# darskkaa/NTIRE-2026-Light-Field-Image-Super-Resolution-Challenge---Track-2-Efficiency

Measured on AMD Instinct MI355X. Metric: 5x5 x4-SR LF patches/sec (32^2->128^2), DistgSSR inference, higher is better.
Workload: dtype f32 (EPI branch stage 1 / 2 and fuse.0: fp32 operands as three exact bf16 terms on the bf16 MFMA pipe, six products, fp32 accumulation -- error against fp64 not above the fp32-MFMA kernels', tests/test_gpu_b3_accuracy.py; 3x3 convs, angular branch, init, head: fp32 MFMA)

## Files before the change

### include/lfsr_hip.h

```cpp
#ifndef LFSR_HIP_H
#define LFSR_HIP_H

#include <stddef.h>
#include <stdint.h>

#ifdef __cplusplus
extern "C" {
#endif

#define LFSR_OK 0
#define LFSR_E_ARG (-1)
#define LFSR_E_WS (-2)

const char* lfsr_version(void);


int lfsr_sai2macpi(const void* in, void* out, int B, int C, int A, int h, int w, int elem_bytes, void* stream);
int lfsr_macpi2sai(const void* in, void* out, int B, int C, int A, int h, int w, int elem_bytes, void* stream);
int lfsr_pixel_shuffle2d(const void* in, void* out, int B, int C, int r, int H, int W, int elem_bytes, void* stream);
int lfsr_pixel_shuffle1d(const void* in, void* out, int B, int C, int f, int H, int W, int elem_bytes, void* stream);
int lfsr_image_extend(const void* in, void* out, int N, int h, int w, int top, int bottom, int left, int right,
                      int elem_bytes, void* stream);
int lfsr_lf_divide(const void* in, void* out, int A, int h0, int w0, int P, int S, int elem_bytes,
                   int* num_u, int* num_v, void* stream);
int lfsr_lf_integrate(const void* in, void* out, int A, int numU, int numV, int pz, int stride, int h, int w,
                      int elem_bytes, void* stream);

int lfsr_lf_crop_tiles(const void* in, void* tiles, int A, int count, int pz, int stride, int elem_bytes, void* stream);
int lfsr_lf_place_tiles(const void* tiles, void* out, int A, int numU, int numV, int first, int count, int stride, int h, int w,
                        int elem_bytes, void* stream);

int lfsr_nchw_to_vcl(const float* in, float* out, int out_stride, int out_choff, int B, int C, int A, int h, int w,
                     int layout, void* stream);
int lfsr_vcl_to_nchw(const float* in, int in_stride, int in_choff, float* out, int B, int C, int A, int h, int w,
                     int layout, void* stream);


int lfsr_pack_conv_weight(const float* w, float* packed, int O, int C, int taps, int perm, int ch, void* stream);
size_t lfsr_packed_weight_floats(int O, int C, int taps);

int lfsr_conv3x3_fwd(const float* x, int x_stride, int x_choff, const float* w_packed,
                     float* y, int y_stride, int y_choff,
                     const float* r1, int r1_stride, int r1_choff, const float* r2, int r2_stride, int r2_choff,
                     int n_img, int h, int w, float slope, void* stream);

int lfsr_pointwise_fwd(const float* x, int x_stride, int x_choff, int cin, const float* w_packed, const float* bias,
                       float* y, int y_stride, int y_choff, int M, int N, float slope, void* stream);

int lfsr_angconv_fwd(const float* x, int x_stride, int x_choff, const float* w1_packed, const float* w2_packed,
                     float* tmp, float* y, int y_stride, int y_choff, int B, int A, int h, int w, float slope, void* stream);

int lfsr_epiconv_fwd(const float* x, int x_stride, int x_choff, const float* w1_packed, const float* w2_packed,
                     float* tmp, float* y, int y_stride, int y_choff, int B, int A, int h, int w, int vertical,
                     float slope, void* stream);

int lfsr_epiconv_hv_fwd(const float* x, int x_stride, int x_choff, const float* w1_packed, const float* w2_packed,
                        float* tmp, float* y, int y_stride, int choff_h, int choff_v, int B, int A, int h, int w,
                        float slope, void* stream);

int lfsr_initconv_fwd(const float* x, const float* w, float* y, int y_stride, int y_choff, int B, int A, int h, int wd,
                      void* stream);

int lfsr_fold_head(const float* w0, const float* b0, const float* w2, float* wf, float* bf, int C, int s, void* stream);
int lfsr_upsample_head_fwd(const float* f, int f_stride, int f_choff, const float* wf, const float* bf,
                           const float* x_lr, float* out, int B, int A, int h, int w, int s, void* stream);

typedef struct lfsr_distgssr lfsr_distgssr;

int lfsr_distgssr_create(lfsr_distgssr** ctx, int A, int scale, int n_group, int n_block, int channels);
void lfsr_distgssr_destroy(lfsr_distgssr* ctx);
size_t lfsr_distgssr_packed_bytes(const lfsr_distgssr* ctx);
int lfsr_distgssr_set_packed(lfsr_distgssr* ctx, void* packed, size_t bytes);
int lfsr_distgssr_load_param(lfsr_distgssr* ctx, const char* key, const float* data, size_t numel, void* stream);
int lfsr_distgssr_finalize(lfsr_distgssr* ctx, void* stream);
int lfsr_distgssr_begin_batched_load(lfsr_distgssr* ctx);
size_t lfsr_distgssr_workspace_bytes(const lfsr_distgssr* ctx, int B, int h, int w);
int lfsr_distgssr_forward(lfsr_distgssr* ctx, const float* x, float* out, int B, int h, int w,
                          void* workspace, size_t workspace_bytes, void* stream);
int lfsr_distgssr_forward_taps(lfsr_distgssr* ctx, const float* x, float* out, int B, int h, int w,
                               void* workspace, size_t workspace_bytes, float* const* taps, void* stream);

size_t lfsr_distgssr_num_params(const lfsr_distgssr* ctx);
int lfsr_distgssr_param_offset(const lfsr_distgssr* ctx, const char* key, size_t* offset, size_t* numel);
size_t lfsr_distgssr_train_workspace_bytes(const lfsr_distgssr* ctx, int B, int h, int w);
int lfsr_distgssr_forward_train(lfsr_distgssr* ctx, const float* x, float* out, int B, int h, int w,
                                void* workspace, size_t workspace_bytes, void* stream);
int lfsr_distgssr_train_saved(const lfsr_distgssr* ctx, int B, int h, int w, int which, int index, size_t* offset_floats, size_t* numel);
int lfsr_distgssr_backward(lfsr_distgssr* ctx, const float* x, const float* dout, int B, int h, int w,
                           void* workspace, size_t workspace_bytes, float* grads, size_t n_grads, void* stream);

size_t lfsr_packed_weight_tr_floats(int O, int C, int taps);
int lfsr_pack_conv_weight_tr(const float* w, float* packed_T, int O, int C, int taps, void* stream);
int lfsr_conv3x3_dgrad(const float* dy, int dy_stride, int dy_choff, const float* wT_packed, float* dx, int dx_stride, int dx_choff,
                       const float* r1, int r1_stride, int r1_choff, const float* act, int act_stride, int act_choff, float act_slope,
                       int n_img, int h, int w, void* stream);
size_t lfsr_conv3x3_wgrad_workspace_floats(int n_img, int h, int w);
int lfsr_conv3x3_wgrad(const float* dy, int dy_stride, int dy_choff, const float* x, int x_stride, int x_choff, float* dw,
                       float* workspace, size_t workspace_floats, int n_img, int h, int w, int accumulate, void* stream);
int lfsr_pointwise_dgrad(const float* dy, int dy_stride, int dy_choff, int cout, const float* wT_packed, float* dx, int dx_stride, int dx_choff, int cin,
                         const float* act, int act_stride, int act_choff, float act_slope, long long M, void* stream);
size_t lfsr_pointwise_wgrad_workspace_floats(long long M, int cout, int cin);
int lfsr_pointwise_wgrad(const float* dy, int dy_stride, int dy_choff, int cout, const float* x, int x_stride, int x_choff, int cin, float* dw,
                         float* workspace, size_t workspace_floats, long long M, int accumulate, void* stream);
int lfsr_upsample_head_dgrad(const float* dout, const float* wf, float* df, float* g16, int B, int A, int h, int w, int s, void* stream);

int lfsr_comm_available(void);
int lfsr_comm_unique_id(void* id128);
int lfsr_comm_init(void** comm, int world, int rank, const void* id128);
int lfsr_comm_destroy(void* comm);
int lfsr_allreduce(void* grads, size_t n, void* comm, void* stream);

#define LFSR_DISTG_NCLASS 6
int lfsr_distgssr_profile(lfsr_distgssr* ctx, int enable);
int lfsr_distgssr_profile_read(lfsr_distgssr* ctx, double* ms, long long* launches);

int lfsr_layernorm_fwd(const float* x, int x_stride, int x_choff, const float* pe, int pe_stride, long long pe_rows, long long pe_div,
                       const float* gamma, const float* beta, float* y, int y_stride, int y_choff, long long M, int C,
                       float eps, void* stream);
int lfsr_linear_fwd(const float* x, int x_stride, int x_choff, int cin, const float* w_packed, const float* bias,
                    const float* res, int res_stride, int res_choff, float* y, int y_stride, int y_choff,
                    long long M, int N, float slope, void* stream);
int lfsr_ffn_fwd(const float* x, int x_stride, int x_choff, const float* w1_packed, const float* w2_packed,
                 const float* res, int res_stride, int res_choff, float* y, int y_stride, int y_choff,
                 long long M, int K1, int H, int N2, float slope, void* stream);
int lfsr_ffn_ln_fwd(const float* x, int x_stride, int x_choff, const float* gamma, const float* beta, float eps,
                    const float* w1_packed, const float* w2_packed, const float* res, int res_stride, int res_choff,
                    float* y, int y_stride, int y_choff, long long M, int K1, int H, int N2, float slope, void* stream);
int lfsr_linear_ln_fwd(const float* x, int x_stride, int x_choff, int K, const float* w_packed, const float* gamma, const float* beta,
                       float eps, int ln_cols, const float* pe, int pe_stride, int pe_rows, int pe_div,
                       float* y, int y_stride, int y_choff, float* y2, int y2_stride, int y2_choff, int split_n,
                       long long M, int N, void* stream);
int lfsr_window_attn_fwd(const float* q, int q_stride, int q_choff, const float* k, int k_stride, int k_choff,
                         const float* v, int v_stride, int v_choff, float* o, int o_stride, int o_choff, int nheads, int hd,
                         int ns0, int ns1, int ns2, long long bs0, long long bs1, long long bs2,
                         int n1, int n2, long long st1, long long st2, int l1, int r1, int l2, int r2, int clip2, void* stream);
int lfsr_conv3x3_n_fwd(const float* x, int x_stride, int x_choff, const float* w_packed, float* y, int y_stride, int y_choff,
                       int n_img, int h, int w, int N, float slope, void* stream);
int lfsr_lft_position_fwd(float* spa_pe, float* ang_pe, int A, int h, int w, int C, void* stream);
int lfsr_upsample_ps_fwd(const float* f, int f_stride, int f_choff, const float* w_packed, float* hr, int B, int A, int h, int w,
                         int s, void* stream);
int lfsr_up_tail_fwd(const float* f, int f_stride, int f_choff, const float* w0_packed, const float* w3, const float* x_lr, float* out,
                     int B, int A, int h, int w, int s, float slope, void* stream);
int lfsr_hr_tail_fwd(const float* hr, const float* w3, const float* x_lr, float* out, int B, int A, int h, int w, int s,
                     float slope, void* stream);

typedef struct lfsr_epit lfsr_epit;
int lfsr_epit_create(lfsr_epit** ctx, int A, int scale, int n_block, int channels);
void lfsr_epit_destroy(lfsr_epit* ctx);
size_t lfsr_epit_packed_bytes(const lfsr_epit* ctx);
int lfsr_epit_set_packed(lfsr_epit* ctx, void* packed, size_t bytes);
int lfsr_epit_load_param(lfsr_epit* ctx, const char* key, const float* data, size_t numel, void* stream);
int lfsr_epit_finalize(lfsr_epit* ctx, void* stream);
size_t lfsr_epit_workspace_bytes(const lfsr_epit* ctx, int B, int h, int w);
int lfsr_epit_forward(lfsr_epit* ctx, const float* x, float* out, int B, int h, int w, void* workspace, size_t workspace_bytes,
                      void* stream);

typedef struct lfsr_lft lfsr_lft;
int lfsr_lft_create(lfsr_lft** ctx, int A, int scale, int n_layer, int channels);
void lfsr_lft_destroy(lfsr_lft* ctx);
size_t lfsr_lft_packed_bytes(const lfsr_lft* ctx);
int lfsr_lft_set_packed(lfsr_lft* ctx, void* packed, size_t bytes);
int lfsr_lft_load_param(lfsr_lft* ctx, const char* key, const float* data, size_t numel, void* stream);
int lfsr_lft_finalize(lfsr_lft* ctx, void* stream);
size_t lfsr_lft_workspace_bytes(const lfsr_lft* ctx, int B, int h, int w);
int lfsr_lft_forward(lfsr_lft* ctx, const float* x, float* out, int B, int h, int w, void* workspace, size_t workspace_bytes,
                     void* stream);

int lfsr_view_metrics(const float* label, const float* out, double* psnr, double* ssim, int B, int A, int H, int W, void* stream);
int lfsr_mask_views(const float* x, float* y, const unsigned char* mask, float fill, int B, int C, int A, int h, int w, void* stream);
int lfsr_mask_views_fill(const float* x, float* y, const unsigned char* mask, const float* fill, int B, int C, int A, int h, int w, void* stream);

int lfsr_ycbcr2rgb_views(const float* y, const float* cbcr, unsigned char* out, int A, int h, int w, const double* minv255,
                         const double* offset, void* stream);

typedef struct lfsr_internet lfsr_internet;
int lfsr_internet_create(lfsr_internet** ctx, int A, int scale, int n_groups, int n_layers);
void lfsr_internet_destroy(lfsr_internet* ctx);
size_t lfsr_internet_packed_bytes(const lfsr_internet* ctx);
int lfsr_internet_set_packed(lfsr_internet* ctx, void* packed, size_t bytes);
int lfsr_internet_load_param(lfsr_internet* ctx, const char* key, const float* data, size_t numel, void* stream);
int lfsr_internet_finalize(lfsr_internet* ctx, void* stream);
size_t lfsr_internet_workspace_bytes(const lfsr_internet* ctx, int B, int h, int w);
int lfsr_internet_forward(lfsr_internet* ctx, const float* x, float* out, int B, int h, int w, void* workspace,
                          size_t workspace_bytes, void* stream);

size_t lfsr_angconv_bwd_workspace_floats(int B, int A, int h, int w);
int lfsr_angconv_bwd(const float* dy, int dy_stride, int dy_choff, const float* y, int y_stride, int y_choff, const float* x, const float* a16,
                     const float* w0, const float* w2, float* dx, float* dw0, float* dw2, float* workspace, size_t workspace_floats,
                     int B, int A, int h, int w, float slope, void* stream);
size_t lfsr_epiconv_hv_bwd_workspace_floats(int B, int A, int h, int w);
int lfsr_epiconv_hv_bwd(const float* dy, int dy_stride, int choff_h, int choff_v, const float* y, int y_stride, int y_choff_h, int y_choff_v,
                        const float* x, const float* e_h, const float* e_v, const float* w0, const float* w2,
                        float* dx, float* dw0, float* dw2, float* workspace, size_t workspace_floats, int B, int A, int h, int w, float slope, void* stream);

#define LFSR_ARITH_DEFAULT 0
#define LFSR_ARITH_F32 1
int lfsr_set_arithmetic(int mode);
int lfsr_get_arithmetic(void);

int lfsr_op_profile(int enable);
long long lfsr_op_profile_read(char* buf, size_t cap);

#ifdef __cplusplus
}
#endif
#endif
```

### ntire-2026-light-field-image-super-resolution-challenge---track-2-efficiency_amd/capi.py

```python
import ctypes as C
import os

import torch

_HERE = os.path.dirname(os.path.abspath(__file__))
LIB_PATH = os.environ.get("LFSR_HIP_LIB") or os.path.join(_HERE, "liblfsr_hip.so")

c_p = C.c_void_p
c_i = C.c_int
c_f = C.c_float
c_sz = C.c_size_t

SIGNATURES = {
    "lfsr_version": (C.c_char_p, []),
    "lfsr_sai2macpi": (c_i, [c_p, c_p, c_i, c_i, c_i, c_i, c_i, c_i, c_p]),
    "lfsr_macpi2sai": (c_i, [c_p, c_p, c_i, c_i, c_i, c_i, c_i, c_i, c_p]),
    "lfsr_pixel_shuffle2d": (c_i, [c_p, c_p, c_i, c_i, c_i, c_i, c_i, c_i, c_p]),
    "lfsr_pixel_shuffle1d": (c_i, [c_p, c_p, c_i, c_i, c_i, c_i, c_i, c_i, c_p]),
    "lfsr_image_extend": (c_i, [c_p, c_p, c_i, c_i, c_i, c_i, c_i, c_i, c_i, c_i, c_p]),
    "lfsr_lf_divide": (c_i, [c_p, c_p, c_i, c_i, c_i, c_i, c_i, c_i, C.POINTER(c_i), C.POINTER(c_i), c_p]),
    "lfsr_lf_integrate": (c_i, [c_p, c_p, c_i, c_i, c_i, c_i, c_i, c_i, c_i, c_i, c_p]),
    "lfsr_lf_crop_tiles": (c_i, [c_p, c_p, c_i, c_i, c_i, c_i, c_i, c_p]),
    "lfsr_lf_place_tiles": (c_i, [c_p, c_p, c_i, c_i, c_i, c_i, c_i, c_i, c_i, c_i, c_i, c_p]),
    "lfsr_nchw_to_vcl": (c_i, [c_p, c_p, c_i, c_i, c_i, c_i, c_i, c_i, c_i, c_i, c_p]),
    "lfsr_vcl_to_nchw": (c_i, [c_p, c_i, c_i, c_p, c_i, c_i, c_i, c_i, c_i, c_i, c_p]),
    "lfsr_pack_conv_weight": (c_i, [c_p, c_p, c_i, c_i, c_i, c_i, c_i, c_p]),
    "lfsr_packed_weight_floats": (c_sz, [c_i, c_i, c_i]),
    "lfsr_conv3x3_fwd": (c_i, [c_p, c_i, c_i, c_p, c_p, c_i, c_i, c_p, c_i, c_i, c_p, c_i, c_i, c_i, c_i, c_i, c_f, c_p]),
    "lfsr_pointwise_fwd": (c_i, [c_p, c_i, c_i, c_i, c_p, c_p, c_p, c_i, c_i, c_i, c_i, c_f, c_p]),
    "lfsr_angconv_fwd": (c_i, [c_p, c_i, c_i, c_p, c_p, c_p, c_p, c_i, c_i, c_i, c_i, c_i, c_i, c_f, c_p]),
    "lfsr_epiconv_fwd": (c_i, [c_p, c_i, c_i, c_p, c_p, c_p, c_p, c_i, c_i, c_i, c_i, c_i, c_i, c_i, c_f, c_p]),
    "lfsr_epiconv_hv_fwd": (c_i, [c_p, c_i, c_i, c_p, c_p, c_p, c_p, c_i, c_i, c_i, c_i, c_i, c_i, c_i, c_f, c_p]),
    "lfsr_initconv_fwd": (c_i, [c_p, c_p, c_p, c_i, c_i, c_i, c_i, c_i, c_i, c_p]),
    "lfsr_fold_head": (c_i, [c_p, c_p, c_p, c_p, c_p, c_i, c_i, c_p]),
    "lfsr_upsample_head_fwd": (c_i, [c_p, c_i, c_i, c_p, c_p, c_p, c_p, c_i, c_i, c_i, c_i, c_i, c_p]),
    "lfsr_distgssr_create": (c_i, [C.POINTER(c_p), c_i, c_i, c_i, c_i, c_i]),
    "lfsr_distgssr_destroy": (None, [c_p]),
    "lfsr_distgssr_packed_bytes": (c_sz, [c_p]),
    "lfsr_distgssr_set_packed": (c_i, [c_p, c_p, c_sz]),
    "lfsr_distgssr_load_param": (c_i, [c_p, C.c_char_p, c_p, c_sz, c_p]),
    "lfsr_distgssr_finalize": (c_i, [c_p, c_p]),
    "lfsr_distgssr_begin_batched_load": (c_i, [c_p]),
    "lfsr_distgssr_workspace_bytes": (c_sz, [c_p, c_i, c_i, c_i]),
    "lfsr_distgssr_forward": (c_i, [c_p, c_p, c_p, c_i, c_i, c_i, c_p, c_sz, c_p]),
    "lfsr_distgssr_forward_taps": (c_i, [c_p, c_p, c_p, c_i, c_i, c_i, c_p, c_sz, C.POINTER(c_p), c_p]),
    "lfsr_distgssr_num_params": (c_sz, [c_p]),
    "lfsr_distgssr_param_offset": (c_i, [c_p, C.c_char_p, C.POINTER(c_sz), C.POINTER(c_sz)]),
    "lfsr_distgssr_train_workspace_bytes": (c_sz, [c_p, c_i, c_i, c_i]),
    "lfsr_distgssr_forward_train": (c_i, [c_p, c_p, c_p, c_i, c_i, c_i, c_p, c_sz, c_p]),
    "lfsr_distgssr_train_saved": (c_i, [c_p, c_i, c_i, c_i, c_i, c_i, C.POINTER(c_sz), C.POINTER(c_sz)]),
    "lfsr_distgssr_backward": (c_i, [c_p, c_p, c_p, c_i, c_i, c_i, c_p, c_sz, c_p, c_sz, c_p]),
    "lfsr_layernorm_fwd": (c_i, [c_p, c_i, c_i, c_p, c_i, C.c_longlong, C.c_longlong, c_p, c_p, c_p, c_i, c_i, C.c_longlong, c_i, c_f, c_p]),
    "lfsr_conv3x3_n_fwd": (c_i, [c_p, c_i, c_i, c_p, c_p, c_i, c_i, c_i, c_i, c_i, c_i, c_f, c_p]),
    "lfsr_lft_position_fwd": (c_i, [c_p, c_p, c_i, c_i, c_i, c_i, c_p]),
    "lfsr_view_metrics": (c_i, [c_p, c_p, c_p, c_p, c_i, c_i, c_i, c_i, c_p]),
    "lfsr_mask_views": (c_i, [c_p, c_p, c_p, c_f, c_i, c_i, c_i, c_i, c_i, c_p]),
    "lfsr_mask_views_fill": (c_i, [c_p, c_p, c_p, c_p, c_i, c_i, c_i, c_i, c_i, c_p]),
    "lfsr_internet_create": (c_i, [C.POINTER(c_p), c_i, c_i, c_i, c_i]),
    "lfsr_internet_destroy": (None, [c_p]),
    "lfsr_internet_packed_bytes": (c_sz, [c_p]),
    "lfsr_internet_set_packed": (c_i, [c_p, c_p, c_sz]),
    "lfsr_internet_load_param": (c_i, [c_p, C.c_char_p, c_p, c_sz, c_p]),
    "lfsr_internet_finalize": (c_i, [c_p, c_p]),
    "lfsr_internet_workspace_bytes": (c_sz, [c_p, c_i, c_i, c_i]),
    "lfsr_internet_forward": (c_i, [c_p, c_p, c_p, c_i, c_i, c_i, c_p, c_sz, c_p]),
    "lfsr_lft_create": (c_i, [C.POINTER(c_p), c_i, c_i, c_i, c_i]),
    "lfsr_lft_destroy": (None, [c_p]),
    "lfsr_lft_packed_bytes": (c_sz, [c_p]),
    "lfsr_lft_set_packed": (c_i, [c_p, c_p, c_sz]),
    "lfsr_lft_load_param": (c_i, [c_p, C.c_char_p, c_p, c_sz, c_p]),
    "lfsr_lft_finalize": (c_i, [c_p, c_p]),
    "lfsr_lft_workspace_bytes": (c_sz, [c_p, c_i, c_i, c_i]),
    "lfsr_lft_forward": (c_i, [c_p, c_p, c_p, c_i, c_i, c_i, c_p, c_sz, c_p]),
    "lfsr_linear_fwd": (c_i, [c_p, c_i, c_i, c_i, c_p, c_p, c_p, c_i, c_i, c_p, c_i, c_i, C.c_longlong, c_i, c_f, c_p]),
    "lfsr_ycbcr2rgb_views": (c_i, [c_p, c_p, c_p, c_i, c_i, c_i, C.POINTER(C.c_double), C.POINTER(C.c_double), c_p]),
    "lfsr_ffn_fwd": (c_i, [c_p, c_i, c_i, c_p, c_p, c_p, c_i, c_i, c_p, c_i, c_i, C.c_longlong, c_i, c_i, c_i, c_f, c_p]),
    "lfsr_ffn_ln_fwd": (c_i, [c_p, c_i, c_i, c_p, c_p, c_f, c_p, c_p, c_p, c_i, c_i, c_p, c_i, c_i, C.c_longlong, c_i, c_i, c_i, c_f, c_p]),
    "lfsr_linear_ln_fwd": (c_i, [c_p, c_i, c_i, c_i, c_p, c_p, c_p, c_f, c_i, c_p, c_i, c_i, c_i, c_p, c_i, c_i, c_p, c_i, c_i, c_i, C.c_longlong, c_i, c_p]),
    "lfsr_window_attn_fwd": (c_i, [c_p, c_i, c_i, c_p, c_i, c_i, c_p, c_i, c_i, c_p, c_i, c_i, c_i, c_i, c_i, c_i, c_i,
                                   C.c_longlong, C.c_longlong, C.c_longlong, c_i, c_i, C.c_longlong, C.c_longlong, c_i, c_i, c_i, c_i, c_i, c_p]),
    "lfsr_upsample_ps_fwd": (c_i, [c_p, c_i, c_i, c_p, c_p, c_i, c_i, c_i, c_i, c_i, c_p]),
    "lfsr_up_tail_fwd": (c_i, [c_p, c_i, c_i, c_p, c_p, c_p, c_p, c_i, c_i, c_i, c_i, c_i, c_f, c_p]),
    "lfsr_hr_tail_fwd": (c_i, [c_p, c_p, c_p, c_p, c_i, c_i, c_i, c_i, c_i, c_f, c_p]),
    "lfsr_epit_create": (c_i, [C.POINTER(c_p), c_i, c_i, c_i, c_i]),
    "lfsr_epit_destroy": (None, [c_p]),
    "lfsr_epit_packed_bytes": (c_sz, [c_p]),
    "lfsr_epit_set_packed": (c_i, [c_p, c_p, c_sz]),
    "lfsr_epit_load_param": (c_i, [c_p, C.c_char_p, c_p, c_sz, c_p]),
    "lfsr_epit_finalize": (c_i, [c_p, c_p]),
    "lfsr_epit_workspace_bytes": (c_sz, [c_p, c_i, c_i, c_i]),
    "lfsr_epit_forward": (c_i, [c_p, c_p, c_p, c_i, c_i, c_i, c_p, c_sz, c_p]),
    "lfsr_packed_weight_tr_floats": (c_sz, [c_i, c_i, c_i]),
    "lfsr_pack_conv_weight_tr": (c_i, [c_p, c_p, c_i, c_i, c_i, c_p]),
    "lfsr_conv3x3_dgrad": (c_i, [c_p, c_i, c_i, c_p, c_p, c_i, c_i, c_p, c_i, c_i, c_p, c_i, c_i, c_f, c_i, c_i, c_i, c_p]),
    "lfsr_conv3x3_wgrad_workspace_floats": (c_sz, [c_i, c_i, c_i]),
    "lfsr_conv3x3_wgrad": (c_i, [c_p, c_i, c_i, c_p, c_i, c_i, c_p, c_p, c_sz, c_i, c_i, c_i, c_i, c_p]),
    "lfsr_pointwise_dgrad": (c_i, [c_p, c_i, c_i, c_i, c_p, c_p, c_i, c_i, c_i, c_p, c_i, c_i, c_f, C.c_longlong, c_p]),
    "lfsr_pointwise_wgrad_workspace_floats": (c_sz, [C.c_longlong, c_i, c_i]),
    "lfsr_pointwise_wgrad": (c_i, [c_p, c_i, c_i, c_i, c_p, c_i, c_i, c_i, c_p, c_p, c_sz, C.c_longlong, c_i, c_p]),
    "lfsr_upsample_head_dgrad": (c_i, [c_p, c_p, c_p, c_p, c_i, c_i, c_i, c_i, c_i, c_p]),
    "lfsr_comm_available": (c_i, []),
    "lfsr_comm_unique_id": (c_i, [c_p]),
    "lfsr_comm_init": (c_i, [C.POINTER(c_p), c_i, c_i, c_p]),
    "lfsr_comm_destroy": (c_i, [c_p]),
    "lfsr_allreduce": (c_i, [c_p, c_sz, c_p, c_p]),
    "lfsr_angconv_bwd_workspace_floats": (c_sz, [c_i, c_i, c_i, c_i]),
    "lfsr_angconv_bwd": (c_i, [c_p, c_i, c_i, c_p, c_i, c_i, c_p, c_p, c_p, c_p, c_p, c_p, c_p, c_p, c_sz, c_i, c_i, c_i, c_i, c_f, c_p]),
    "lfsr_epiconv_hv_bwd_workspace_floats": (c_sz, [c_i, c_i, c_i, c_i]),
    "lfsr_epiconv_hv_bwd": (c_i, [c_p, c_i, c_i, c_i, c_p, c_i, c_i, c_i, c_p, c_p, c_p, c_p, c_p, c_p, c_p, c_p, c_p, c_sz, c_i, c_i, c_i, c_i, c_f, c_p]),
    "lfsr_set_arithmetic": (c_i, [c_i]),
    "lfsr_get_arithmetic": (c_i, []),
    "lfsr_op_profile": (c_i, [c_i]),
    "lfsr_op_profile_read": (C.c_longlong, [C.c_char_p, c_sz]),
    "lfsr_distgssr_profile": (c_i, [c_p, c_i]),
    "lfsr_distgssr_profile_read": (c_i, [c_p, C.POINTER(C.c_double), C.POINTER(C.c_longlong)]),
}

_lib = None


class LfsrError(RuntimeError):
    pass


def load():
    global _lib
    if _lib is None:
        if not os.path.exists(LIB_PATH):
            raise LfsrError(f"{LIB_PATH} not built: run `python -c 'import __graft_entry__ as g; g.build()'` "
                            "(there is no CPU fallback for the HIP path)")
        lib = C.CDLL(LIB_PATH)
        for name, (res, args) in SIGNATURES.items():
            fn = getattr(lib, name)
            fn.restype = res
            fn.argtypes = args
        _lib = lib
    return _lib


def check(rc, what):
    if rc != 0:
        if rc == -1:
            msg = "bad argument"
        elif rc == -2:
            msg = "workspace too small"
        else:
            msg = f"HIP error {-rc - 1000}"
        raise LfsrError(f"{what}: {msg} (rc={rc})")


def stream_ptr():
    return C.c_void_p(torch.cuda.current_stream().cuda_stream)


def dev_ptr(t, what="tensor"):
    if not isinstance(t, torch.Tensor) or not t.is_cuda:
        raise LfsrError(f"{what} must be a CUDA/ROCm tensor: the HIP path has no CPU fallback")
    if not t.is_contiguous():
        raise LfsrError(f"{what} must be contiguous")
    return C.c_void_p(t.data_ptr())


def _elem(t):
    eb = t.element_size()
    if eb not in (2, 4):
        raise LfsrError(f"unsupported element size {eb}")
    return eb


ARITH_DEFAULT, ARITH_F32 = 0, 1


def set_arithmetic(mode):
    check(load().lfsr_set_arithmetic(int(mode)), "set_arithmetic")


def op_profile(enable):
    check(load().lfsr_op_profile(int(bool(enable))), "op_profile")


def op_profile_read():
    lib = load()
    cap = 1 << 18
    buf = C.create_string_buffer(cap)
    need = lib.lfsr_op_profile_read(buf, cap)
    if need < 0:
        check(int(need), "op_profile_read")
    if need > cap:
        raise LfsrError(f"op_profile_read: table of {need} bytes truncated")
    out = {}
    for line in buf.value.decode().splitlines():
        op, a, b, ms, n = line.split()
        out[(op, int(a), int(b))] = (float(ms), int(n))
    return out



def sai2macpi(x, A):
    lib = load()
    B, Cc, Hh, Ww = x.shape
    out = torch.empty_like(x)
    check(lib.lfsr_sai2macpi(dev_ptr(x), dev_ptr(out), B, Cc, A, Hh // A, Ww // A, _elem(x), stream_ptr()), "sai2macpi")
    return out


def macpi2sai(x, A):
    lib = load()
    B, Cc, Hh, Ww = x.shape
    out = torch.empty_like(x)
    check(lib.lfsr_macpi2sai(dev_ptr(x), dev_ptr(out), B, Cc, A, Hh // A, Ww // A, _elem(x), stream_ptr()), "macpi2sai")
    return out


def pixel_shuffle2d(x, r):
    lib = load()
    B, Crr, H, W = x.shape
    Cc = Crr // (r * r)
    out = torch.empty((B, Cc, H * r, W * r), dtype=x.dtype, device=x.device)
    check(lib.lfsr_pixel_shuffle2d(dev_ptr(x), dev_ptr(out), B, Cc, r, H, W, _elem(x), stream_ptr()), "pixel_shuffle2d")
    return out


def pixel_shuffle1d(x, f):
    lib = load()
    B, fC, H, W = x.shape
    Cc = fC // f
    out = torch.empty((B, Cc, H, W * f), dtype=x.dtype, device=x.device)
    check(lib.lfsr_pixel_shuffle1d(dev_ptr(x), dev_ptr(out), B, Cc, f, H, W, _elem(x), stream_ptr()), "pixel_shuffle1d")
    return out


def image_extend(im, bdr):
    lib = load()
    h, w = im.shape[-2:]
    N = im.numel() // (h * w) if h * w else 0
    out = torch.empty(tuple(im.shape[:-2]) + (h + bdr[0] + bdr[1], w + bdr[2] + bdr[3]), dtype=im.dtype, device=im.device)
    check(lib.lfsr_image_extend(dev_ptr(im), dev_ptr(out), N, h, w, bdr[0], bdr[1], bdr[2], bdr[3], _elem(im), stream_ptr()), "image_extend")
    return out


def lf_divide(data, A, P, S):
    lib = load()
    if data.dim() != 2:
        raise LfsrError("LFdivide expects a 2-D (A*h0, A*w0) mosaic")
    h0, w0 = data.shape[0] // A, data.shape[1] // A
    nu, nv = c_i(0), c_i(0)
    check(lib.lfsr_lf_divide(None, None, A, h0, w0, P, S, _elem(data), C.byref(nu), C.byref(nv), None), "lf_divide(count)")
    out = torch.empty((nu.value, nv.value, A * P, A * P), dtype=data.dtype, device=data.device)
    check(lib.lfsr_lf_divide(dev_ptr(data), dev_ptr(out), A, h0, w0, P, S, _elem(data), None, None, stream_ptr()), "lf_divide")
    return out


def lf_integrate(sub, A, pz, stride, h, w):
    lib = load()
    if sub.dim() == 6:
        n1, n2 = sub.shape[:2]
        sub = sub.permute(0, 1, 2, 4, 3, 5).reshape(n1, n2, A * pz, A * pz).contiguous()
    n1, n2 = sub.shape[:2]
    out = torch.empty((A, A, h, w), dtype=sub.dtype, device=sub.device)
    check(lib.lfsr_lf_integrate(dev_ptr(sub), dev_ptr(out), A, n1, n2, pz, stride, h, w, _elem(sub), stream_ptr()), "lf_integrate")
    return out


def lf_crop_tiles(sub, A, pz, stride):
    lib = load()
    n = sub.shape[0]
    if sub.shape[-1] != A * pz or sub.shape[-2] != A * pz or sub.numel() != n * A * pz * A * pz:
        raise LfsrError(f"lf_crop_tiles: bad patch tensor {tuple(sub.shape)} for A={A} pz={pz}")
    sub = sub.contiguous()
    out = torch.empty((n, A, A, stride, stride), dtype=sub.dtype, device=sub.device)
    check(lib.lfsr_lf_crop_tiles(dev_ptr(sub), dev_ptr(out), A, n, pz, stride, _elem(sub), stream_ptr()), "lf_crop_tiles")
    return out


def lf_place_tiles(tiles, out, A, numU, numV, first, stride):
    lib = load()
    tiles = tiles.contiguous()
    if not out.is_contiguous() or out.dtype != tiles.dtype or out.shape[0] != A or out.shape[1] != A:
        raise LfsrError("lf_place_tiles: bad output tensor")
    check(lib.lfsr_lf_place_tiles(dev_ptr(tiles), dev_ptr(out), A, numU, numV, first, tiles.shape[0], stride, out.shape[2], out.shape[3], _elem(tiles), stream_ptr()),
          "lf_place_tiles")
    return out


def nchw_to_vcl(x, A, layout, out=None, choff=0):
    lib = load()
    B, Cc, Hh, Ww = x.shape
    h, w = Hh // A, Ww // A
    if out is None:
        out = torch.empty((B * A * A * h * w, Cc), dtype=torch.float32, device=x.device)
    check(lib.lfsr_nchw_to_vcl(dev_ptr(x), dev_ptr(out), out.shape[1], choff, B, Cc, A, h, w, layout, stream_ptr()), "nchw_to_vcl")
    return out


def vcl_to_nchw(v, B, Cc, A, h, w, layout, choff=0):
    lib = load()
    out = torch.empty((B, Cc, A * h, A * w), dtype=torch.float32, device=v.device)
    check(lib.lfsr_vcl_to_nchw(dev_ptr(v), v.shape[1], choff, dev_ptr(out), B, Cc, A, h, w, layout, stream_ptr()), "vcl_to_nchw")
    return out


def pack_conv_weight(w, perm=0, ch=0):
    lib = load()
    O, Cc = w.shape[:2]
    taps = w.numel() // (O * Cc)
    n = lib.lfsr_packed_weight_floats(O, Cc, taps)
    out = torch.empty(n, dtype=torch.float32, device=w.device)
    check(lib.lfsr_pack_conv_weight(dev_ptr(w), dev_ptr(out), O, Cc, taps, perm, ch, stream_ptr()), "pack_conv_weight")
    return out



def max_patches_per_launch(A, h, w, widest_row_floats, limit=1 << 31):
    per_patch = A * A * h * w * widest_row_floats * 4
    return max(1, (limit - 1) // per_patch)


def _forward_in_chunks(fwd, x, nmax):
    return torch.cat([fwd(x[i:i + nmax]) for i in range(0, x.shape[0], nmax)], 0)


class GraphedForward:

    def __init__(self, rt):
        self.rt = rt
        self.graphs = {}

    def __call__(self, x):
        key = (tuple(x.shape), x.device, x.dtype)
        g = self.graphs.get(key)
        if g is None:
            static_x = x.clone()
            side = torch.cuda.Stream(device=x.device)
            side.wait_stream(torch.cuda.current_stream())
            with torch.cuda.stream(side):
                for _ in range(2):
                    self.rt.forward(static_x)
            torch.cuda.current_stream().wait_stream(side)
            graph = torch.cuda.CUDAGraph()
            with torch.cuda.graph(graph):
                static_y = self.rt.forward(static_x)
            g = self.graphs[key] = (graph, static_x, static_y)
        graph, static_x, static_y = g
        static_x.copy_(x)
        graph.replay()
        return static_y



class DistgSSRRuntime:

    def __init__(self, A, scale, n_group=4, n_block=4, channels=64):
        self.lib = load()
        self.A, self.scale = A, scale
        ctx = c_p()
        check(self.lib.lfsr_distgssr_create(C.byref(ctx), A, scale, n_group, n_block, channels), "distgssr_create")
        self.ctx = ctx
        self.packed = None
        self.ws = {}
        self.loaded_version = None
        self.train_generation = 0

    def __del__(self):
        try:
            if getattr(self, "ctx", None):
                self.lib.lfsr_distgssr_destroy(self.ctx)
                self.ctx = None
        except Exception:
            pass

    def load_state(self, named_tensors, device, fanout=None, batched=False):
        nbytes = self.lib.lfsr_distgssr_packed_bytes(self.ctx)
        if self.packed is None or self.packed.device != device:
            self.packed = torch.empty(nbytes, dtype=torch.uint8, device=device)
        check(self.lib.lfsr_distgssr_set_packed(self.ctx, dev_ptr(self.packed), nbytes), "distgssr_set_packed")
        cur = torch.cuda.current_stream(device)
        st = stream_ptr()
        keep = []
        if batched:
            check(self.lib.lfsr_distgssr_begin_batched_load(self.ctx), "distgssr_begin_batched_load")
        if fanout:
            fork = torch.cuda.Event()
            fork.record(cur)
            for s in fanout:
                s.wait_event(fork)
        for i, (k, t) in enumerate(named_tensors):
            t = t.detach()
            if t.dtype != torch.float32:
                t = t.float()
            t = t.contiguous()
            sp = C.c_void_p(fanout[i % len(fanout)].cuda_stream) if fanout else st
            keep.append(t)
            check(self.lib.lfsr_distgssr_load_param(self.ctx, k.encode(), dev_ptr(t, k), t.numel(), sp), f"distgssr_load_param({k})")
        if fanout:
            for s in fanout:
                e = torch.cuda.Event()
                e.record(s)
                cur.wait_event(e)
        check(self.lib.lfsr_distgssr_finalize(self.ctx, st), "distgssr_finalize")

    def _workspace(self, B, h, w, device):
        key = (B, h, w, device)
        if key not in self.ws:
            self.ws.clear()
            n = self.lib.lfsr_distgssr_workspace_bytes(self.ctx, B, h, w)
            self.ws[key] = torch.empty(n, dtype=torch.uint8, device=device)
        return self.ws[key]

    def num_params(self):
        return self.lib.lfsr_distgssr_num_params(self.ctx)

    def param_span(self, key):
        off, n = c_sz(0), c_sz(0)
        check(self.lib.lfsr_distgssr_param_offset(self.ctx, key.encode(), C.byref(off), C.byref(n)), f"param_offset({key})")
        return off.value, n.value

    def _train_workspace(self, B, h, w, device):
        key = ("train", B, h, w, device)
        if key not in self.ws:
            self.ws.clear()
            n = self.lib.lfsr_distgssr_train_workspace_bytes(self.ctx, B, h, w)
            self.ws[key] = torch.empty(n, dtype=torch.uint8, device=device)
        return self.ws[key]

    def forward_train(self, x):
        B, c1, Hh, Ww = x.shape
        if c1 != 1 or Hh % self.A or Ww % self.A or x.dtype != torch.float32:
            raise LfsrError(f"bad training input {tuple(x.shape)} {x.dtype}")
        h, w = Hh // self.A, Ww // self.A
        x = x.contiguous()
        out = torch.empty((B, 1, Hh * self.scale, Ww * self.scale), dtype=torch.float32, device=x.device)
        ws = self._train_workspace(B, h, w, x.device)
        check(self.lib.lfsr_distgssr_forward_train(self.ctx, dev_ptr(x), dev_ptr(out), B, h, w, dev_ptr(ws), ws.numel(), stream_ptr()),
              "distgssr_forward_train")
        self.train_generation += 1
        return out

    def backward(self, x, dout, grads=None):
        B, _, Hh, Ww = x.shape
        h, w = Hh // self.A, Ww // self.A
        n = self.num_params()
        if grads is None:
            grads = torch.empty(n, dtype=torch.float32, device=x.device)
        ws = self._train_workspace(B, h, w, x.device)
        dout = dout.contiguous()
        if dout.dtype != torch.float32:
            dout = dout.float()
        check(self.lib.lfsr_distgssr_backward(self.ctx, dev_ptr(x.contiguous()), dev_ptr(dout), B, h, w, dev_ptr(ws), ws.numel(),
                                              dev_ptr(grads), n, stream_ptr()), "distgssr_backward")
        return grads

    def train_saved(self, x, which, index):
        B, _, Hh, Ww = x.shape
        h, w = Hh // self.A, Ww // self.A
        off, n = c_sz(0), c_sz(0)
        check(self.lib.lfsr_distgssr_train_saved(self.ctx, B, h, w, which, index, C.byref(off), C.byref(n)), "train_saved")
        ws = self._train_workspace(B, h, w, x.device).view(torch.float32)
        return ws[off.value:off.value + n.value]

    PROFILE_CLASSES = ("conv3x3", "angconv", "epiconv", "pointwise", "init_conv", "upsample_head")

    def profile(self, enable):
        check(self.lib.lfsr_distgssr_profile(self.ctx, int(enable)), "distgssr_profile")

    def profile_read(self):
        ms = (C.c_double * 6)()
        n = (C.c_longlong * 6)()
        check(self.lib.lfsr_distgssr_profile_read(self.ctx, ms, n), "distgssr_profile_read")
        return {k: (ms[i], n[i]) for i, k in enumerate(self.PROFILE_CLASSES)}

    def forward(self, x, taps=None):
        B, c1, Hh, Ww = x.shape
        if c1 != 1 or Hh % self.A or Ww % self.A:
            raise LfsrError(f"bad input shape {tuple(x.shape)} for angRes {self.A}")
        if x.dtype != torch.float32:
            raise LfsrError("DistgSSR HIP path computes in fp32; got " + str(x.dtype))
        h, w = Hh // self.A, Ww // self.A
        x = x.contiguous()
        if taps is None and B > max_patches_per_launch(self.A, h, w, 160, 1 << 30):
            return _forward_in_chunks(self.forward, x, max_patches_per_launch(self.A, h, w, 160, 1 << 30))
        out = torch.empty((B, 1, Hh * self.scale, Ww * self.scale), dtype=torch.float32, device=x.device)
        ws = self._workspace(B, h, w, x.device)
        if taps is None:
            check(self.lib.lfsr_distgssr_forward(self.ctx, dev_ptr(x), dev_ptr(out), B, h, w, dev_ptr(ws), ws.numel(), stream_ptr()),
                  "distgssr_forward")
            return out
        bufs = []
        arr = (c_p * 5)()
        for i in range(5):
            if taps[i]:
                t = torch.empty((B, 144 if i == 4 else 64, Hh, Ww), dtype=torch.float32, device=x.device)
                arr[i] = t.data_ptr()
            else:
                t = None
                arr[i] = None
            bufs.append(t)
        check(self.lib.lfsr_distgssr_forward_taps(self.ctx, dev_ptr(x), dev_ptr(out), B, h, w, dev_ptr(ws), ws.numel(), arr, stream_ptr()),
              "distgssr_forward_taps")
        return out, bufs



def _opt(t):
    return dev_ptr(t) if t is not None else None


def conv3x3(x, w_packed, n_img, h, w, slope=1.0, res1=None, res2=None, out=None, out_choff=0, x_choff=0):
    lib = load()
    if out is None:
        out = torch.empty((n_img * h * w, 64), dtype=torch.float32, device=x.device)
    check(lib.lfsr_conv3x3_fwd(dev_ptr(x), x.shape[1], x_choff, dev_ptr(w_packed), dev_ptr(out), out.shape[1], out_choff,
                               _opt(res1), res1.shape[1] if res1 is not None else 0, 0,
                               _opt(res2), res2.shape[1] if res2 is not None else 0, 0,
                               n_img, h, w, slope, stream_ptr()), "conv3x3_fwd")
    return out


def pointwise(x, cin, w_packed, N, slope=1.0, bias=None, out=None, out_choff=0, x_choff=0):
    lib = load()
    M = x.shape[0]
    if out is None:
        out = torch.empty((M, N), dtype=torch.float32, device=x.device)
    check(lib.lfsr_pointwise_fwd(dev_ptr(x), x.shape[1], x_choff, cin, dev_ptr(w_packed), _opt(bias), dev_ptr(out), out.shape[1], out_choff,
                                 M, N, slope, stream_ptr()), "pointwise_fwd")
    return out


def angconv(x, w1p, w2p, B, A, h, w, slope, out, out_choff, tmp=None):
    lib = load()
    if tmp is None:
        tmp = torch.empty((B * h * w, 16), dtype=torch.float32, device=x.device)
    check(lib.lfsr_angconv_fwd(dev_ptr(x), x.shape[1], 0, dev_ptr(w1p), dev_ptr(w2p), dev_ptr(tmp), dev_ptr(out), out.shape[1], out_choff,
                               B, A, h, w, slope, stream_ptr()), "angconv_fwd")
    return out


def epiconv(x, w1p, w2p, B, A, h, w, vertical, slope, out, out_choff, tmp=None):
    lib = load()
    if tmp is None:
        tmp = torch.empty((B * A * h * w, 32), dtype=torch.float32, device=x.device)
    check(lib.lfsr_epiconv_fwd(dev_ptr(x), x.shape[1], 0, dev_ptr(w1p), dev_ptr(w2p), dev_ptr(tmp), dev_ptr(out), out.shape[1], out_choff,
                               B, A, h, w, int(vertical), slope, stream_ptr()), "epiconv_fwd")
    return out


def epiconv_hv(x, w1p, w2p, B, A, h, w, slope, out, choff_h, choff_v):
    lib = load()
    tmp = torch.empty((B * A * h * w, 32), dtype=torch.float32, device=x.device)
    check(lib.lfsr_epiconv_hv_fwd(dev_ptr(x), x.shape[1], 0, dev_ptr(w1p), dev_ptr(w2p), dev_ptr(tmp), dev_ptr(out), out.shape[1], choff_h, choff_v,
                                  B, A, h, w, slope, stream_ptr()), "epiconv_hv_fwd")
    return out


def initconv(x, w, A):
    lib = load()
    B, _, Hh, Ww = x.shape
    h, wd = Hh // A, Ww // A
    out = torch.empty((B * A * A * h * wd, 64), dtype=torch.float32, device=x.device)
    check(lib.lfsr_initconv_fwd(dev_ptr(x), dev_ptr(w), dev_ptr(out), 64, 0, B, A, h, wd, stream_ptr()), "initconv_fwd")
    return out


def upsample_head(f, w0, b0, w2, x_lr, A, s):
    lib = load()
    B, _, Hh, Ww = x_lr.shape
    h, w = Hh // A, Ww // A
    wf = torch.empty(s * s * 64, dtype=torch.float32, device=f.device)
    bf = torch.empty(s * s, dtype=torch.float32, device=f.device)
    check(lib.lfsr_fold_head(dev_ptr(w0), _opt(b0), dev_ptr(w2), dev_ptr(wf), dev_ptr(bf), 64, s, stream_ptr()), "fold_head")
    out = torch.empty((B, 1, Hh * s, Ww * s), dtype=torch.float32, device=f.device)
    check(lib.lfsr_upsample_head_fwd(dev_ptr(f), f.shape[1], 0, dev_ptr(wf), dev_ptr(bf), dev_ptr(x_lr), dev_ptr(out), B, A, h, w, s, stream_ptr()),
          "upsample_head_fwd")
    return out



class ModelRuntime:

    def __init__(self, name, A, scale, *create_args):
        self.lib = load()
        self.name, self.A, self.scale = name, A, scale
        self._f = lambda fn: getattr(self.lib, f"lfsr_{name}_{fn}")
        ctx = c_p()
        check(self._f("create")(C.byref(ctx), A, scale, *create_args), f"{name}_create")
        self.ctx = ctx
        self.packed = None
        self.ws = {}

    def __del__(self):
        try:
            if getattr(self, "ctx", None):
                self._f("destroy")(self.ctx)
                self.ctx = None
        except Exception:
            pass

    def load_state(self, named_tensors, device):
        nbytes = self._f("packed_bytes")(self.ctx)
        if self.packed is None or self.packed.device != device:
            self.packed = torch.empty(nbytes, dtype=torch.uint8, device=device)
        check(self._f("set_packed")(self.ctx, dev_ptr(self.packed), nbytes), f"{self.name}_set_packed")
        st = stream_ptr()
        for k, t in named_tensors:
            t = t.detach().float().contiguous()
            check(self._f("load_param")(self.ctx, k.encode(), dev_ptr(t, k), t.numel(), st), f"{self.name}_load_param({k})")
        check(self._f("finalize")(self.ctx, st), f"{self.name}_finalize")

    def forward(self, x):
        B, c1, Hh, Ww = x.shape
        if c1 != 1 or Hh % self.A or Ww % self.A:
            raise LfsrError(f"bad input shape {tuple(x.shape)} for angRes {self.A}")
        if x.dtype != torch.float32:
            raise LfsrError(f"{self.name} HIP path computes in fp32; got {x.dtype}")
        h, w = Hh // self.A, Ww // self.A
        x = x.contiguous()
        if B > max_patches_per_launch(self.A, h, w, 256):
            return _forward_in_chunks(self.forward, x, max_patches_per_launch(self.A, h, w, 256))
        out = torch.empty((B, 1, Hh * self.scale, Ww * self.scale), dtype=torch.float32, device=x.device)
        key = (B, h, w, x.device)
        if key not in self.ws:
            self.ws.clear()
            self.ws[key] = torch.empty(self._f("workspace_bytes")(self.ctx, B, h, w), dtype=torch.uint8, device=x.device)
        ws = self.ws[key]
        check(self._f("forward")(self.ctx, dev_ptr(x), dev_ptr(out), B, h, w, dev_ptr(ws), ws.numel(), stream_ptr()), f"{self.name}_forward")
        return out



def pack_conv_weight_T(w):
    lib = load()
    O, Cc = w.shape[:2]
    taps = w.numel() // (O * Cc)
    out = torch.empty(lib.lfsr_packed_weight_tr_floats(O, Cc, taps), dtype=torch.float32, device=w.device)
    check(lib.lfsr_pack_conv_weight_tr(dev_ptr(w), dev_ptr(out), O, Cc, taps, stream_ptr()), "pack_conv_weight_T")
    return out


def conv3x3_dgrad(dy, wT_packed, n_img, h, w, res1=None, act=None, act_slope=1.0):
    lib = load()
    dx = torch.empty((n_img * h * w, 64), dtype=torch.float32, device=dy.device)
    check(lib.lfsr_conv3x3_dgrad(dev_ptr(dy), dy.shape[1], 0, dev_ptr(wT_packed), dev_ptr(dx), 64, 0,
                                 _opt(res1), res1.shape[1] if res1 is not None else 0, 0,
                                 _opt(act), act.shape[1] if act is not None else 0, 0, act_slope, n_img, h, w, stream_ptr()), "conv3x3_dgrad")
    return dx


def conv3x3_wgrad(dy, x, n_img, h, w, dw=None):
    lib = load()
    acc = dw is not None
    if dw is None:
        dw = torch.empty((64, 64, 3, 3), dtype=torch.float32, device=dy.device)
    ws = torch.empty(lib.lfsr_conv3x3_wgrad_workspace_floats(n_img, h, w), dtype=torch.float32, device=dy.device)
    check(lib.lfsr_conv3x3_wgrad(dev_ptr(dy), dy.shape[1], 0, dev_ptr(x), x.shape[1], 0, dev_ptr(dw), dev_ptr(ws), ws.numel(), n_img, h, w, int(acc),
                                 stream_ptr()), "conv3x3_wgrad")
    return dw


def pointwise_dgrad(dy, wT_packed, cin, act=None, act_slope=1.0):
    lib = load()
    M = dy.shape[0]
    dx = torch.empty((M, cin), dtype=torch.float32, device=dy.device)
    check(lib.lfsr_pointwise_dgrad(dev_ptr(dy), dy.shape[1], 0, 64, dev_ptr(wT_packed), dev_ptr(dx), cin, 0, cin,
                                   _opt(act), act.shape[1] if act is not None else 0, 0, act_slope, M, stream_ptr()), "pointwise_dgrad")
    return dx


def pointwise_wgrad(dy, x, cout, cin):
    lib = load()
    M = dy.shape[0]
    dw = torch.empty((cout, cin), dtype=torch.float32, device=dy.device)
    ws = torch.empty(lib.lfsr_pointwise_wgrad_workspace_floats(M, cout, cin), dtype=torch.float32, device=dy.device)
    check(lib.lfsr_pointwise_wgrad(dev_ptr(dy), dy.shape[1], 0, cout, dev_ptr(x), x.shape[1], 0, cin, dev_ptr(dw), dev_ptr(ws), ws.numel(), M, 0,
                                   stream_ptr()), "pointwise_wgrad")
    return dw


class RcclComm:

    def __init__(self, world, rank, exchange=None):
        self.lib = load()
        if not self.lib.lfsr_comm_available():
            raise LfsrError("RCCL not found (librccl.so): lfsr_allreduce is unavailable on this host")
        buf = C.create_string_buffer(128)
        if rank == 0:
            check(self.lib.lfsr_comm_unique_id(buf), "comm_unique_id")
        raw = bytes(buf.raw)
        if world > 1:
            if exchange is None:
                raise LfsrError("world > 1 needs an `exchange` callable to ship rank 0's unique id")
            raw = exchange(raw)
        comm = c_p()
        check(self.lib.lfsr_comm_init(C.byref(comm), world, rank, C.create_string_buffer(raw, 128)), "comm_init")
        self.comm, self.world = comm, world

    def allreduce_(self, t):
        if t.dtype != torch.float32:
            raise LfsrError("lfsr_allreduce carries fp32 buckets")
        check(self.lib.lfsr_allreduce(dev_ptr(t), t.numel(), self.comm, stream_ptr()), "allreduce")
        return t

    def close(self):
        if getattr(self, "comm", None):
            self.lib.lfsr_comm_destroy(self.comm)
            self.comm = None


def angconv_bwd(dy, dy_choff, y, y_choff, x, a16, w0, w2, dx, B, A, h, w, slope=0.1):
    lib = load()
    ws = torch.empty(lib.lfsr_angconv_bwd_workspace_floats(B, A, h, w), dtype=torch.float32, device=x.device)
    dw0, dw2 = torch.empty_like(w0), torch.empty_like(w2)
    check(lib.lfsr_angconv_bwd(dev_ptr(dy), dy.shape[1], dy_choff, _opt(y), y.shape[1] if y is not None else 0, y_choff, dev_ptr(x), dev_ptr(a16),
                               dev_ptr(w0.contiguous()), dev_ptr(w2.contiguous()), dev_ptr(dx), dev_ptr(dw0), dev_ptr(dw2), dev_ptr(ws), ws.numel(), B, A, h, w, slope,
                               stream_ptr()), "angconv_bwd")
    return dw0, dw2


def epiconv_hv_bwd(dy, choff_h, choff_v, y, y_choff_h, y_choff_v, x, e_h, e_v, w0, w2, dx, B, A, h, w, slope=0.1):
    lib = load()
    ws = torch.empty(lib.lfsr_epiconv_hv_bwd_workspace_floats(B, A, h, w), dtype=torch.float32, device=x.device)
    dw0, dw2 = torch.empty_like(w0), torch.empty_like(w2)
    check(lib.lfsr_epiconv_hv_bwd(dev_ptr(dy), dy.shape[1], choff_h, choff_v, _opt(y), y.shape[1] if y is not None else 0, y_choff_h, y_choff_v, dev_ptr(x),
                                  dev_ptr(e_h), dev_ptr(e_v), dev_ptr(w0.contiguous()), dev_ptr(w2.contiguous()), dev_ptr(dx), dev_ptr(dw0), dev_ptr(dw2),
                                  dev_ptr(ws), ws.numel(), B, A, h, w, slope, stream_ptr()), "epiconv_hv_bwd")
    return dw0, dw2
```

### ntire-2026-light-field-image-super-resolution-challenge---track-2-efficiency_amd/csrc/ang_fused.hip

```cpp
#include "lfsr_internal.h"

typedef float f32x4a __attribute__((ext_vector_type(4)));

namespace {

constexpr int W1ROW = 68;
constexpr int TROW = 20;

struct AngArgs {
  const float* X; int x_stride; int x_choff;
  const float* W1;
  const float* W2;
  float* T;
  float* Y; int y_stride; int y_choff;
  int B, A, H, W;
  float slope;
};

__global__ __launch_bounds__(512) void k_ang_fused(AngArgs p) {
  extern __shared__ __attribute__((aligned(16))) float sm[];
  const int AA = p.A * p.A, HW = p.H * p.W, M = p.B * HW;
  float* sW1 = sm;
  float* sW2 = sm + AA * 16 * W1ROW;
  float* sT = sW2 + 16 * AA * 16;
  const int tid = threadIdx.x, lane = tid & 63, wave = tid >> 6, nwave = blockDim.x >> 6;
  const int i = lane & 15, kq = lane >> 4;

  const int ngroups = (M + 15) / 16, gstride = (int)gridDim.x * nwave;
  const int g0 = (int)blockIdx.x * nwave + wave;
  const long long tstep = (long long)HW * p.x_stride;
  float4 fb[2][5][4];
  auto load_row = [&](int g, int u, float4 (*f)[4]) {
    const int m = g * 16 + i;
    const bool ok = m < M;
    const int mb = ok ? m / HW : 0, myx = ok ? m - mb * HW : 0;
    const float* src = p.X + ((long long)mb * AA * HW + myx) * p.x_stride + p.x_choff + 4 * kq;
#pragma unroll
    for (int v = 0; v < 5; ++v)
#pragma unroll
      for (int j = 0; j < 4; ++j)
        f[v][j] = (ok && v < p.A) ? *reinterpret_cast<const float4*>(src + (u * p.A + v) * tstep + 16 * j) : make_float4(0.f, 0.f, 0.f, 0.f);
  };
  {
    float4 wv[13];
#pragma unroll
    for (int q = 0; q < 13; ++q) {
      const int idx = tid + q * 512, row = idx >> 4, c = idx & 15, tap = row >> 4, n = row & 15;
      wv[q] = idx < AA * 256 ? *reinterpret_cast<const float4*>(p.W1 + ((long long)tap * 32 + n) * 64 + c * 4) : make_float4(0.f, 0.f, 0.f, 0.f);
    }
    float4 w2v[4];
#pragma unroll
    for (int q = 0; q < 4; ++q) {
      const int idx = tid + q * 512;
      w2v[q] = idx < AA * 64 ? reinterpret_cast<const float4*>(p.W2)[idx] : make_float4(0.f, 0.f, 0.f, 0.f);
    }
    if (g0 < ngroups) load_row(g0, 0, fb[0]);
#pragma unroll
    for (int q = 0; q < 13; ++q) {
      const int idx = tid + q * 512;
      if (idx < AA * 256) *reinterpret_cast<float4*>(sW1 + (idx >> 4) * W1ROW + (idx & 15) * 4) = wv[q];
    }
#pragma unroll
    for (int q = 0; q < 4; ++q) {
      const int idx = tid + q * 512;
      if (idx < AA * 64) reinterpret_cast<float4*>(sW2)[idx] = w2v[q];
    }
  }
  __syncthreads();

  float* st = sT + wave * 16 * TROW;
  const float* b1 = sW1 + i * W1ROW + 4 * kq;
  const float* b2 = sW2 + i * 16 + 4 * kq;

  for (int g = g0; g < ngroups; g += gstride) {
    const int m = g * 16 + i;
    const bool ok = m < M;
    const int mb = ok ? m / HW : 0, myx = ok ? m - mb * HW : 0;
    if (g != g0) load_row(g, 0, fb[0]);
    f32x4a acc = {0.f, 0.f, 0.f, 0.f};
#pragma unroll
    for (int u = 0; u < 5; ++u) {
      if (u >= p.A) break;
      if (u + 1 < p.A) load_row(g, u + 1, fb[(u + 1) & 1]);
#pragma unroll
      for (int v = 0; v < 5; ++v) {
        if (v >= p.A) break;
        const float* bt = b1 + (u * p.A + v) * 16 * W1ROW;
#pragma unroll
        for (int j = 0; j < 4; ++j) {
          const float4 b = *reinterpret_cast<const float4*>(bt + 16 * j);
          const float4 a = fb[u & 1][v][j];
          acc = __builtin_amdgcn_mfma_f32_16x16x4f32(a.x, b.x, acc, 0, 0, 0);
          acc = __builtin_amdgcn_mfma_f32_16x16x4f32(a.y, b.y, acc, 0, 0, 0);
          acc = __builtin_amdgcn_mfma_f32_16x16x4f32(a.z, b.z, acc, 0, 0, 0);
          acc = __builtin_amdgcn_mfma_f32_16x16x4f32(a.w, b.w, acc, 0, 0, 0);
        }
      }
    }
#pragma unroll
    for (int r = 0; r < 4; ++r) {
      float v = acc[r];
      v = v >= 0.f ? v : v * p.slope;
      st[(4 * kq + r) * TROW + i] = v;
    }
    const int b_i = ok ? mb : 0;
    const long long dbase = ok ? (long long)b_i * AA * HW + myx : -1;
    __builtin_amdgcn_wave_barrier();
    const float4 a2 = *reinterpret_cast<const float4*>(st + i * TROW + 4 * kq);
    if (ok) *reinterpret_cast<float4*>(p.T + (long long)m * 16 + 4 * kq) = a2;
    __builtin_amdgcn_wave_barrier();
    for (int view = 0; view < AA; ++view) {
      const float4 b = *reinterpret_cast<const float4*>(b2 + view * 256);
      f32x4a o = {0.f, 0.f, 0.f, 0.f};
      o = __builtin_amdgcn_mfma_f32_16x16x4f32(a2.x, b.x, o, 0, 0, 0);
      o = __builtin_amdgcn_mfma_f32_16x16x4f32(a2.y, b.y, o, 0, 0, 0);
      o = __builtin_amdgcn_mfma_f32_16x16x4f32(a2.z, b.z, o, 0, 0, 0);
      o = __builtin_amdgcn_mfma_f32_16x16x4f32(a2.w, b.w, o, 0, 0, 0);
#pragma unroll
      for (int r = 0; r < 4; ++r) {
        float v = o[r];
        v = v >= 0.f ? v : v * p.slope;
        st[(4 * kq + r) * TROW + i] = v;
      }
      __builtin_amdgcn_wave_barrier();
      const float4 z = *reinterpret_cast<const float4*>(st + i * TROW + 4 * kq);
      __builtin_amdgcn_wave_barrier();
      if (ok) *reinterpret_cast<float4*>(p.Y + (dbase + (long long)view * HW) * p.y_stride + p.y_choff + 4 * kq) = z;
    }
  }
}

}

size_t lfsr_ang_fused_smem(int A, int waves) {
  const int AA = A * A;
  return (size_t)(AA * 16 * W1ROW + 16 * AA * 16 + waves * 16 * TROW) * 4;
}

bool lfsr_ang_fused_ok(int A) { return A >= 1 && A <= 5 && lfsr_ang_fused_smem(A, 8) <= 160 * 1024; }

int lfsr_ang_fused_launch(const float* x, int x_stride, int x_choff, const float* w1_packed, const float* w2_packed, float* t, float* y,
                          int y_stride, int y_choff, int B, int A, int h, int w, float slope, hipStream_t st) {
  if (!lfsr_ang_fused_ok(A)) return LFSR_E_ARG;
  static std::atomic<bool> attr_set[64];
  int dev = 0;
  if (hipGetDevice(&dev) != hipSuccess || dev < 0 || dev >= 64) return LFSR_E_ARG;
  if (!attr_set[dev]) {
    hipError_t e = hipFuncSetAttribute(reinterpret_cast<const void*>(k_ang_fused), hipFuncAttributeMaxDynamicSharedMemorySize, 160 * 1024);
    if (e != hipSuccess) return LFSR_HIP_ERR(e);
    attr_set[dev] = true;
  }
  AngArgs p{};
  p.X = x; p.x_stride = x_stride; p.x_choff = x_choff; p.W1 = w1_packed; p.W2 = w2_packed; p.T = t;
  p.Y = y; p.y_stride = y_stride; p.y_choff = y_choff; p.B = B; p.A = A; p.H = h; p.W = w; p.slope = slope;
  const long long ngroups = ((long long)B * h * w + 15) / 16;
  const int waves = 8;
  long long grid = (ngroups + waves - 1) / waves;
  if (grid > 256) grid = 256;
  hipLaunchKernelGGL(k_ang_fused, dim3((unsigned)grid), dim3(waves * 64), lfsr_ang_fused_smem(A, waves), st, p);
  LFSR_CHECK_LAUNCH();
  return LFSR_OK;
}
```

### ntire-2026-light-field-image-super-resolution-challenge---track-2-efficiency_amd/csrc/distgssr.cpp

```cpp
#include <cstring>
#include <map>
#include <string>
#include <vector>

#include "lfsr_internal.h"

namespace {
struct Slot {
  size_t off = 0;
  size_t floats = 0;
  size_t numel = 0;
  int O = 0, C = 0, T = 0, perm = 0, ch = 0;
  bool raw = false, loaded = false;
  int kindT = 0;
  size_t offT = 0, floatsT = 0;
  size_t grad_off = 0;
};
inline size_t align64(size_t f) { return (f + 63) / 64 * 64; }
}

struct lfsr_distgssr {
  int A, s, G, NB, C;
  std::map<std::string, Slot> slots;
  std::vector<std::string> order;
  size_t n_params = 0;
  size_t packed_floats = 0, off_wf = 0, off_bf = 0;
  float* packed = nullptr;
  bool finalized = false;
  bool batch_mode = false;
  std::vector<LfsrPackDesc> d_gen, d_c3, d_epi, d_epib, uploaded;
  LfsrPackDesc* table_dev = nullptr;
  size_t table_cap = 0;
  hipStream_t side = nullptr;
  hipEvent_t ev_fork = nullptr, ev_join = nullptr, ev_a = nullptr, ev_b = nullptr;
  bool profiling = false;
  struct Ev { int cls; hipEvent_t a, b; };
  bool profile_all = true;
  int sample_stride = 1;
  long long sample_ctr = 0;
  std::vector<Ev> evs;
  std::vector<hipEvent_t> free_evs;
  hipEvent_t get_ev() {
    if (!free_evs.empty()) { hipEvent_t e = free_evs.back(); free_evs.pop_back(); return e; }
    hipEvent_t e = nullptr;
    (void)hipEventCreate(&e);
    return e;
  }

  void add(const std::string& k, int O, int Cc, int T, int perm, int ch, bool raw, int kindT = 0) {
    Slot sl;
    sl.O = O; sl.C = Cc; sl.T = T; sl.perm = perm; sl.ch = ch; sl.raw = raw; sl.kindT = kindT;
    sl.numel = (size_t)O * Cc * T;
    sl.floats = raw ? sl.numel : lfsr_packed_weight_floats(O, Cc, T);
    sl.off = packed_floats;
    packed_floats += align64(sl.floats);
    if (kindT == 1 || kindT == 2) sl.floatsT = (size_t)T * ((Cc + 31) / 32 * 32) * O;
    if (kindT == 1 && O == 64 && Cc == 64 && T == 9) sl.floatsT += LFSR_CONV3_WINO_FLOATS;
    if (kindT == 3 || kindT == 4) sl.floatsT = (size_t)(O / (kindT == 3 ? 16 : 32)) * ((Cc + 31) / 32 * 32) * (kindT == 3 ? 16 : 32);
    if (kindT) { sl.offT = packed_floats; packed_floats += align64(sl.floatsT); }
    sl.grad_off = n_params;
    n_params += sl.numel;
    slots[k] = sl;
    order.push_back(k);
  }
  const float* wT(const std::string& k) const { return packed + slots.at(k).offT; }
  const float* w(const std::string& k) const { return packed + slots.at(k).off; }
};

extern "C" {

int lfsr_distgssr_create(lfsr_distgssr** out, int A, int scale, int n_group, int n_block, int channels) {
  if (!out || A <= 0 || A > 15 || (scale != 2 && scale != 3 && scale != 4) || n_group <= 0 || n_block <= 0 || channels != 64) return LFSR_E_ARG;
  lfsr_distgssr* c = new lfsr_distgssr();
  c->A = A; c->s = scale; c->G = n_group; c->NB = n_block; c->C = channels;
  const int AA = A * A;
  c->add("init_conv.weight", 64, 1, 9, 0, 0, true);
  for (int g = 0; g < n_group; ++g) {
    for (int b = 0; b < n_block; ++b) {
      std::string p = "disentg.Group." + std::to_string(g) + ".Block." + std::to_string(b) + ".";
      c->add(p + "SpaConv.0.weight", 64, 64, 9, 0, 0, false, 1);
      c->add(p + "SpaConv.2.weight", 64, 64, 9, 0, 0, false, 1);
      c->add(p + "AngConv.0.weight", 16, 64, AA, 0, 0, false, 2);
      c->add(p + "AngConv.2.weight", 16 * AA, 16, 1, 1, 16, false, 3);
      c->add(p + "EPIConv.0.weight", 32, 64, AA, 0, 0, false, 2);
      c->add(p + "EPIConv.2.weight", 32 * A, 32, 1, 0, 0, false, 4);
      c->add(p + "fuse.0.weight", 64, 144, 1, 0, 0, false, 2);
      c->add(p + "fuse.2.weight", 64, 64, 9, 0, 0, false, 1);
    }
    c->add("disentg.Group." + std::to_string(g) + ".conv.weight", 64, 64, 9, 0, 0, false, 1);
  }
  c->add("disentg.conv.weight", 64, 64, 9, 0, 0, false, 1);
  c->add("upsample.0.weight", 64 * scale * scale, 64, 1, 0, 0, true);
  c->add("upsample.0.bias", 64 * scale * scale, 1, 1, 0, 0, true);
  c->add("upsample.2.weight", 1, 64, 1, 0, 0, true);
  c->off_wf = c->packed_floats; c->packed_floats += align64((size_t)scale * scale * 64);
  c->off_bf = c->packed_floats; c->packed_floats += align64((size_t)scale * scale);
  *out = c;
  return LFSR_OK;
}

void lfsr_distgssr_destroy(lfsr_distgssr* c) {
  if (!c) return;
  for (auto& e : c->evs) { (void)hipEventDestroy(e.a); (void)hipEventDestroy(e.b); }
  for (auto e : c->free_evs) (void)hipEventDestroy(e);
  if (c->table_dev) (void)hipFree(c->table_dev);
  if (c->ev_fork) (void)hipEventDestroy(c->ev_fork);
  if (c->ev_join) (void)hipEventDestroy(c->ev_join);
  if (c->ev_a) (void)hipEventDestroy(c->ev_a);
  if (c->ev_b) (void)hipEventDestroy(c->ev_b);
  if (c->side) (void)hipStreamDestroy(c->side);
  delete c;
}

int lfsr_distgssr_begin_batched_load(lfsr_distgssr* c) {
  if (!c) return LFSR_E_ARG;
  c->batch_mode = true;
  c->d_gen.clear(); c->d_c3.clear(); c->d_epi.clear(); c->d_epib.clear();
  return LFSR_OK;
}

int lfsr_distgssr_profile(lfsr_distgssr* c, int enable) {
  if (!c) return LFSR_E_ARG;
  for (auto& e : c->evs) { c->free_evs.push_back(e.a); c->free_evs.push_back(e.b); }
  c->evs.clear();
  c->profiling = enable != 0;
  c->profile_all = enable == 1;
  c->sample_stride = enable == 3 ? 4 : 1;
  c->sample_ctr = 0;
  return LFSR_OK;
}

int lfsr_distgssr_profile_read(lfsr_distgssr* c, double* ms, long long* launches) {
  if (!c || !ms || !launches) return LFSR_E_ARG;
  for (int i = 0; i < LFSR_DISTG_NCLASS; ++i) { ms[i] = 0.0; launches[i] = 0; }
  for (auto& e : c->evs) {
    hipError_t err = hipEventSynchronize(e.b);
    if (err != hipSuccess) return LFSR_HIP_ERR(err);
    float t = 0.f;
    err = hipEventElapsedTime(&t, e.a, e.b);
    if (err != hipSuccess) return LFSR_HIP_ERR(err);
    ms[e.cls] += t;
    launches[e.cls] += 1;
    c->free_evs.push_back(e.a); c->free_evs.push_back(e.b);
  }
  c->evs.clear();
  return LFSR_OK;
}

size_t lfsr_distgssr_packed_bytes(const lfsr_distgssr* c) { return c ? c->packed_floats * sizeof(float) : 0; }

int lfsr_distgssr_set_packed(lfsr_distgssr* c, void* packed, size_t bytes) {
  if (!c || !packed || bytes < c->packed_floats * sizeof(float) || ((uintptr_t)packed & 15)) return LFSR_E_ARG;
  c->packed = (float*)packed;
  c->finalized = false;
  for (auto& kv : c->slots) kv.second.loaded = false;
  return LFSR_OK;
}

int lfsr_distgssr_load_param(lfsr_distgssr* c, const char* key, const float* data, size_t numel, void* stream) {
  if (!c || !key || !data || !c->packed) return LFSR_E_ARG;
  auto it = c->slots.find(key);
  if (it == c->slots.end()) return LFSR_E_ARG;
  Slot& sl = it->second;
  if (numel != sl.numel) return LFSR_E_ARG;
  c->finalized = false;
  if (sl.raw) {
    hipError_t e = hipMemcpyAsync(c->packed + sl.off, data, numel * sizeof(float), hipMemcpyDeviceToDevice, lfsr_stream(stream));
    if (e != hipSuccess) return LFSR_HIP_ERR(e);
  } else if (c->batch_mode && (lfsr_conv3_variant_mask() == LFSR_W_WINO4 || !(sl.O == 64 && sl.C == 64 && sl.T == 9))) {
    auto pad32 = [](int v) { return (v + 31) / 32 * 32; };
    float* dst = c->packed + sl.off;
    float* tdst = c->packed + sl.offT;
    const bool c3 = sl.O == 64 && sl.C == 64 && sl.T == 9 && sl.perm == 0;
    if (c3) c->d_c3.push_back(LfsrPackDesc{data, dst, dst + LFSR_CONV3_DIRECT_FLOATS + LFSR_CONV3_WINO2_FLOATS, 0, 64, 64, 9, 64, 0, 0, 0});
    else {
      c->d_gen.push_back(LfsrPackDesc{data, dst, nullptr, 0, sl.O, sl.C, sl.T, pad32(sl.O), sl.perm, sl.ch, 0});
      if (sl.O == 32 && sl.C == 64 && sl.T == 25 && sl.perm == 0) {
        c->d_epi.push_back(LfsrPackDesc{dst, dst + 25 * 32 * 64, nullptr, 0, 32, 64, 25, 32, 0, 0, 0});
        c->d_epib.push_back(LfsrPackDesc{dst, dst + 25 * 32 * 64 + LFSR_EPI_WINO_FLOATS, nullptr, 0, 32, 64, 25, 32, 0, 0, 0});
      }
      if (sl.O == 160 && sl.C == 32 && sl.T == 1 && sl.perm == 0) c->d_epib.push_back(LfsrPackDesc{dst, dst + 160 * 32, nullptr, 1, 160, 32, 1, 160, 0, 0, 0});
    }
    if (sl.kindT == 1 && c3) c->d_c3.push_back(LfsrPackDesc{data, tdst, tdst + LFSR_CONV3_DIRECT_FLOATS + LFSR_CONV3_WINO2_FLOATS, 0, 64, 64, 9, 64, 0, 0, 1});
    else if (sl.kindT == 1) c->d_gen.push_back(LfsrPackDesc{data, tdst, nullptr, 1, sl.O, sl.C, sl.T, pad32(sl.C), 0, 0, 1});
    if (sl.kindT == 2) c->d_gen.push_back(LfsrPackDesc{data, tdst, nullptr, 1, sl.O, sl.C, sl.T, pad32(sl.C), 0, 0, 0});
    if (sl.kindT == 3) c->d_gen.push_back(LfsrPackDesc{data, tdst, nullptr, 2, sl.O, sl.C, 1, pad32(sl.C), 1, 16, 0});
    if (sl.kindT == 4) c->d_gen.push_back(LfsrPackDesc{data, tdst, nullptr, 2, sl.O, sl.C, 1, pad32(sl.C), 0, 32, 0});
  } else {
    const int vmask = lfsr_conv3_variant_mask();
    int rc = lfsr_pack_conv_weight_m(data, c->packed + sl.off, sl.O, sl.C, sl.T, sl.perm, sl.ch, vmask, stream);
    if (rc) return rc;
    float* tdst = c->packed + sl.offT;
    if (sl.kindT == 1) rc = lfsr_pack_weight_T_m(data, tdst, sl.O, sl.C, sl.T, 1, vmask, lfsr_stream(stream));
    if (sl.kindT == 2) rc = lfsr_pack_weight_T(data, tdst, sl.O, sl.C, sl.T, 0, lfsr_stream(stream));
    if (sl.kindT == 3) rc = lfsr_pack_weight_chunkT(data, tdst, sl.O, sl.C, 16, 1, lfsr_stream(stream));
    if (sl.kindT == 4) rc = lfsr_pack_weight_chunkT(data, tdst, sl.O, sl.C, 32, 0, lfsr_stream(stream));
    if (rc) return rc;
  }
  sl.loaded = true;
  return LFSR_OK;
}

int lfsr_distgssr_finalize(lfsr_distgssr* c, void* stream) {
  if (!c || !c->packed) return LFSR_E_ARG;
  for (auto& kv : c->slots)
    if (!kv.second.loaded) return LFSR_E_ARG;
  if (c->batch_mode) {
    c->batch_mode = false;
    std::vector<LfsrPackDesc> all(c->d_gen);
    all.insert(all.end(), c->d_c3.begin(), c->d_c3.end());
    all.insert(all.end(), c->d_epi.begin(), c->d_epi.end());
    all.insert(all.end(), c->d_epib.begin(), c->d_epib.end());
    bool same = all.size() == c->uploaded.size();
    for (size_t i = 0; same && i < all.size(); ++i) same = memcmp(&all[i], &c->uploaded[i], sizeof(LfsrPackDesc)) == 0;
    if (!same) {
      if (all.size() > c->table_cap) {
        if (c->table_dev) (void)hipFree(c->table_dev);
        c->table_dev = nullptr; c->table_cap = 0;
        hipError_t e = hipMalloc(reinterpret_cast<void**>(&c->table_dev), (all.size() + 64) * sizeof(LfsrPackDesc));
        if (e != hipSuccess) return LFSR_HIP_ERR(e);
        c->table_cap = all.size() + 64;
      }
      c->uploaded = all;
      hipError_t e = hipMemcpyAsync(c->table_dev, c->uploaded.data(), all.size() * sizeof(LfsrPackDesc), hipMemcpyHostToDevice, lfsr_stream(stream));
      if (e != hipSuccess) return LFSR_HIP_ERR(e);
    }
    const int ng = (int)c->d_gen.size(), n3 = (int)c->d_c3.size(), ne = (int)c->d_epi.size(), nb3 = (int)c->d_epib.size();
    int rcb = lfsr_pack_generic_batch(c->table_dev, ng, lfsr_stream(stream));
    if (!rcb) rcb = lfsr_pack_conv3_raw_wino4_batch(c->table_dev + ng, n3, lfsr_stream(stream));
    if (!rcb) rcb = lfsr_pack_epi_wino_batch(c->table_dev + ng + n3, ne, lfsr_stream(stream));
    if (!rcb) rcb = lfsr_pack_epi_b3_batch(c->table_dev + ng + n3 + ne, nb3, lfsr_stream(stream));
    if (rcb) return rcb;
  }
  int rc = lfsr_fold_head(c->w("upsample.0.weight"), c->w("upsample.0.bias"), c->w("upsample.2.weight"),
                          c->packed + c->off_wf, c->packed + c->off_bf, 64, c->s, stream);
  if (rc) return rc;
  c->finalized = true;
  return LFSR_OK;
}

static void ws_layout(const lfsr_distgssr* c, int B, int h, int w, size_t off[8], size_t* total) {
  const size_t npix = (size_t)B * c->A * c->A * h * w;
  size_t o = 0;
  for (int i = 0; i < 5; ++i) { off[i] = o; o += align64(npix * 64); }
  off[5] = o; o += align64(npix * 144);
  off[6] = o; o += align64((size_t)B * h * w * 16);
  off[7] = o; o += align64((size_t)B * c->A * h * w * 32);
  *total = o;
}

size_t lfsr_distgssr_workspace_bytes(const lfsr_distgssr* c, int B, int h, int w) {
  if (!c || B <= 0 || h <= 0 || w <= 0) return 0;
  size_t off[8], tot;
  ws_layout(c, B, h, w, off, &tot);
  return tot * sizeof(float);
}

int lfsr_distgssr_forward_taps(lfsr_distgssr* c, const float* x, float* out, int B, int h, int w, void* workspace,
                               size_t workspace_bytes, float* const* taps, void* stream) {
  if (!c || !x || !out || !workspace || B <= 0 || h <= 0 || w <= 0 || !c->finalized) return LFSR_E_ARG;
  if ((uintptr_t)workspace & 15) return LFSR_E_ARG;
  size_t off[8], tot;
  ws_layout(c, B, h, w, off, &tot);
  if (workspace_bytes < tot * sizeof(float)) return LFSR_E_WS;
  if ((long long)B * c->A * c->A * h * w * 160 * 4 >= (1LL << 30)) return LFSR_E_ARG;
  float* ws = (float*)workspace;
  float* pool[4] = {ws + off[0], ws + off[1], ws + off[2], ws + off[3]};
  float* T = ws + off[4];
  float* CAT = ws + off[5];
  float* A16 = ws + off[6];
  float* E32 = ws + off[7];
  const int A = c->A, AA = A * A, nimg = B * AA;
  const float L = 0.1f;
  int rc;
#define RC(call) do { rc = (call); if (rc) return rc; } while (0)
#define PROF(cls, call)                                                              \
  do {                                                                               \
    if (c->profiling && (c->profile_all || ((cls) == 0 && (c->sample_stride <= 1 || (c->sample_ctr++ % c->sample_stride) == 0)))) { \
      lfsr_distgssr::Ev ev{cls, c->get_ev(), c->get_ev()};                           \
      (void)hipEventRecord(ev.a, lfsr_stream(stream));                                     \
      rc = (call);                                                                   \
      (void)hipEventRecord(ev.b, lfsr_stream(stream));                                     \
      c->evs.push_back(ev);                                                          \
    } else {                                                                         \
      rc = (call);                                                                   \
    }                                                                                \
    if (rc) return rc;                                                               \
  } while (0)
  auto tap = [&](int which, const float* buf, int stride, int C) -> int {
    if (!taps || !taps[which]) return LFSR_OK;
    return lfsr_vcl_to_nchw(buf, stride, 0, taps[which], B, C, A, h, w, 1, stream);
  };
  auto pick = [&](const float* a, const float* b2, const float* c2) -> float* {
    for (int i = 0; i < 4; ++i)
      if (pool[i] != a && pool[i] != b2 && pool[i] != c2) return pool[i];
    return nullptr;
  };
  auto conv = [&](const float* in, const std::string& key, float* o, int ostride, int ochoff, const float* res, float slope) -> int {
    return lfsr_conv3x3_fwd(in, 64, 0, c->w(key), o, ostride, ochoff, res, 64, 0, nullptr, 0, 0, nimg, h, w, slope, stream);
  };

  float* F0 = pool[0];
  PROF(4, lfsr_initconv_fwd(x, c->w("init_conv.weight"), F0, 64, 0, B, A, h, w, stream));
  RC(tap(0, F0, 64, 64));
  const float* cur = F0;
  for (int g = 0; g < c->G; ++g) {
    const float* gin = cur;
    for (int b = 0; b < c->NB; ++b) {
      std::string p = "disentg.Group." + std::to_string(g) + ".Block." + std::to_string(b) + ".";
      float* o = pick(F0, gin, cur);
      PROF(0, conv(cur, p + "SpaConv.0.weight", T, 64, 0, nullptr, L));
      PROF(0, conv(T, p + "SpaConv.2.weight", CAT, 144, 0, nullptr, L));
      PROF(1, lfsr_angconv_fwd(cur, 64, 0, c->w(p + "AngConv.0.weight"), c->w(p + "AngConv.2.weight"), A16, CAT, 144, 64, B, A, h, w, L, stream));
      PROF(2, lfsr_epiconv_hv_fwd(cur, 64, 0, c->w(p + "EPIConv.0.weight"), c->w(p + "EPIConv.2.weight"), E32, CAT, 144, 80, 112, B, A, h, w, L, stream));
      if (g == 0 && b == 0) RC(tap(4, CAT, 144, 144));
      PROF(3, lfsr_pointwise_fwd(CAT, 144, 0, 144, c->w(p + "fuse.0.weight"), nullptr, T, 64, 0, nimg * h * w, 64, L, stream));
      PROF(0, conv(T, p + "fuse.2.weight", o, 64, 0, cur, 1.0f));
      cur = o;
      if (g == 0 && b == 0) RC(tap(1, cur, 64, 64));
    }
    float* o = pick(F0, gin, cur);
    PROF(0, conv(cur, "disentg.Group." + std::to_string(g) + ".conv.weight", o, 64, 0, gin, 1.0f));
    cur = o;
    if (g == 0) RC(tap(2, cur, 64, 64));
  }
  {
    float* o = pick(F0, cur, cur);
    PROF(0, conv(cur, "disentg.conv.weight", o, 64, 0, F0, 1.0f));
    cur = o;
    RC(tap(3, cur, 64, 64));
  }
  PROF(5, lfsr_upsample_head_fwd(cur, 64, 0, c->packed + c->off_wf, c->packed + c->off_bf, x, out, B, A, h, w, c->s, stream));
#undef RC
#undef PROF
  return LFSR_OK;
}

int lfsr_distgssr_forward(lfsr_distgssr* c, const float* x, float* out, int B, int h, int w, void* workspace,
                          size_t workspace_bytes, void* stream) {
  return lfsr_distgssr_forward_taps(c, x, out, B, h, w, workspace, workspace_bytes, nullptr, stream);
}

}

namespace {
struct TrainWs {
  float *F0, *D;
  std::vector<float*> S1, CAT, A16, EH, EV, FZ, OUT, GOUT;
  float *g[4], *dF, *dS1, *dCAT, *dA16, *dE32, *dE32V, *G16, *XG9, *P[4], *PA, *small;
  size_t pfloats;
  size_t total;
};

size_t max_partial_floats(const lfsr_distgssr* c, int B, int h, int w) {
  const int A = c->A, AA = A * A;
  const int npix = B * AA * h * w, nlr = B * h * w, nepi = B * A * h * w;
  size_t m = 0;
  auto up = [&](size_t v) { if (v > m) m = v; };
  up(lfsr_wgrad_partial_floats(npix, 9, 64, 64));
  up((size_t)256 * 9 * 64 * 64);
  up(lfsr_branch_bwd_partial_floats(B, A, h, w));
  up(lfsr_wgrad_partial_floats(npix, 1, 64, 144));
  up(lfsr_wgrad_partial_floats(nlr, AA, 16, 64));
  up(lfsr_wgrad_partial_floats(nlr, AA, 16, 16));
  up(lfsr_wgrad_partial_floats(nepi, AA, 32, 64));
  up(lfsr_wgrad_partial_floats(nepi, A, 32, 32));
  up(lfsr_wgrad_partial_floats(npix, 1, 16, 64));
  up(lfsr_wgrad_partial_floats(npix, 1, 64, 16));
  return m;
}

void train_layout(const lfsr_distgssr* c, int B, int h, int w, float* base, TrainWs& t) {
  const int A = c->A, AA = A * A, nb = c->G * c->NB;
  const size_t npix = (size_t)B * AA * h * w, nlr = (size_t)B * h * w, nepi = (size_t)B * A * h * w;
  size_t o = 0;
  auto take = [&](size_t floats) { float* p = base ? base + o : nullptr; o += align64(floats); return p; };
  t.F0 = take(npix * 64); t.D = take(npix * 64);
  t.S1.resize(nb); t.CAT.resize(nb); t.A16.resize(nb); t.EH.resize(nb); t.EV.resize(nb); t.FZ.resize(nb); t.OUT.resize(nb); t.GOUT.resize(c->G);
  for (int i = 0; i < nb; ++i) {
    t.S1[i] = take(npix * 64); t.CAT[i] = take(npix * 144); t.A16[i] = take(nlr * 16);
    t.EH[i] = take(nepi * 32); t.EV[i] = take(nepi * 32); t.FZ[i] = take(npix * 64); t.OUT[i] = take(npix * 64);
  }
  for (int g = 0; g < c->G; ++g) t.GOUT[g] = take(npix * 64);
  for (int i = 0; i < 4; ++i) t.g[i] = take(npix * 64);
  t.dF = take(npix * 64); t.dS1 = take(npix * 64); t.dCAT = take(npix * 144);
  t.dA16 = take(nlr * 16); t.dE32 = take(nepi * 32); t.dE32V = take(nepi * 32); t.G16 = take(npix * 16); t.XG9 = take(npix * 16);
  t.pfloats = max_partial_floats(c, B, h, w);
  for (int i = 0; i < 4; ++i) t.P[i] = take(t.pfloats);
  t.PA = take(lfsr_branch_bwd_partial_floats(B, c->A, h, w));
  t.small = take(64 * 1024);
  t.total = o;
}
}

extern "C" {

size_t lfsr_distgssr_num_params(const lfsr_distgssr* c) { return c ? c->n_params : 0; }

int lfsr_distgssr_param_offset(const lfsr_distgssr* c, const char* key, size_t* off, size_t* numel) {
  if (!c || !key) return LFSR_E_ARG;
  auto it = c->slots.find(key);
  if (it == c->slots.end()) return LFSR_E_ARG;
  if (off) *off = it->second.grad_off;
  if (numel) *numel = it->second.numel;
  return LFSR_OK;
}

size_t lfsr_distgssr_train_workspace_bytes(const lfsr_distgssr* c, int B, int h, int w) {
  if (!c || B <= 0 || h <= 0 || w <= 0) return 0;
  TrainWs t;
  train_layout(c, B, h, w, nullptr, t);
  return t.total * sizeof(float);
}

int lfsr_distgssr_train_saved(const lfsr_distgssr* c, int B, int h, int w, int which, int index, size_t* offset_floats, size_t* numel) {
  if (!c || B <= 0 || h <= 0 || w <= 0 || index < 0 || index >= c->G * c->NB || !offset_floats || !numel) return LFSR_E_ARG;
  TrainWs t;
  float* const base = reinterpret_cast<float*>(uintptr_t(4096));
  train_layout(c, B, h, w, base, t);
  const size_t npix = (size_t)B * c->A * c->A * h * w, nlr = (size_t)B * h * w, nepi = (size_t)B * c->A * h * w;
  const float* p = nullptr; size_t n = 0;
  switch (which) {
    case 0: p = t.S1[index]; n = npix * 64; break;
    case 1: p = t.CAT[index]; n = npix * 144; break;
    case 2: p = t.A16[index]; n = nlr * 16; break;
    case 3: p = t.EH[index]; n = nepi * 32; break;
    case 4: p = t.EV[index]; n = nepi * 32; break;
    case 5: p = t.FZ[index]; n = npix * 64; break;
    case 6: p = t.OUT[index]; n = npix * 64; break;
    default: return LFSR_E_ARG;
  }
  *offset_floats = (size_t)(p - base); *numel = n;
  return LFSR_OK;
}

int lfsr_distgssr_forward_train(lfsr_distgssr* c, const float* x, float* out, int B, int h, int w, void* workspace, size_t workspace_bytes, void* stream) {
  if (!c || !x || !out || !workspace || B <= 0 || h <= 0 || w <= 0 || !c->finalized || ((uintptr_t)workspace & 15)) return LFSR_E_ARG;
  TrainWs t;
  train_layout(c, B, h, w, (float*)workspace, t);
  if (workspace_bytes < t.total * sizeof(float)) return LFSR_E_WS;
  if ((long long)B * c->A * c->A * h * w * 160 * 4 >= (1LL << 30)) return LFSR_E_ARG;
  const int A = c->A, AA = A * A, nimg = B * AA;
  const float L = 0.1f;
  hipStream_t st = lfsr_stream(stream);
  int rc;
#define RC(call) do { rc = (call); if (rc) return rc; } while (0)
  auto conv = [&](const float* in, const std::string& key, float* o, int ostride, const float* res, float slope) -> int {
    return lfsr_conv3x3_fwd(in, 64, 0, c->w(key), o, ostride, 0, res, 64, 0, nullptr, 0, 0, nimg, h, w, slope, stream);
  };
  RC(lfsr_initconv_fwd(x, c->w("init_conv.weight"), t.F0, 64, 0, B, A, h, w, stream));
  const float* cur = t.F0;
  for (int g = 0; g < c->G; ++g) {
    const float* gin = cur;
    for (int b = 0; b < c->NB; ++b) {
      const int i = g * c->NB + b;
      std::string p = "disentg.Group." + std::to_string(g) + ".Block." + std::to_string(b) + ".";
      RC(conv(cur, p + "SpaConv.0.weight", t.S1[i], 64, nullptr, L));
      RC(conv(t.S1[i], p + "SpaConv.2.weight", t.CAT[i], 144, nullptr, L));
      RC(lfsr_angconv_fwd(cur, 64, 0, c->w(p + "AngConv.0.weight"), c->w(p + "AngConv.2.weight"), t.A16[i], t.CAT[i], 144, 64, B, A, h, w, L, stream));
      if (lfsr_epi_fused_ok(A, h, w)) {
        RC(lfsr_epi_fused_launch(cur, 64, 0, c->w(p + "EPIConv.0.weight"), c->w(p + "EPIConv.2.weight"), t.CAT[i], 144, 80, 112, t.EH[i], t.EV[i], B, A, h, w, 3, L, st));
      } else {
        RC(lfsr_epiconv_gather(cur, 64, 0, c->w(p + "EPIConv.0.weight"), c->w(p + "EPIConv.2.weight"), t.EH[i], t.CAT[i], 144, 80, B, A, h, w, 0, L, st));
        RC(lfsr_epiconv_gather(cur, 64, 0, c->w(p + "EPIConv.0.weight"), c->w(p + "EPIConv.2.weight"), t.EV[i], t.CAT[i], 144, 112, B, A, h, w, 1, L, st));
      }
      RC(lfsr_pointwise_fwd(t.CAT[i], 144, 0, 144, c->w(p + "fuse.0.weight"), nullptr, t.FZ[i], 64, 0, nimg * h * w, 64, L, stream));
      RC(conv(t.FZ[i], p + "fuse.2.weight", t.OUT[i], 64, cur, 1.0f));
      cur = t.OUT[i];
    }
    RC(conv(cur, "disentg.Group." + std::to_string(g) + ".conv.weight", t.GOUT[g], 64, gin, 1.0f));
    cur = t.GOUT[g];
  }
  RC(conv(cur, "disentg.conv.weight", t.D, 64, t.F0, 1.0f));
  RC(lfsr_upsample_head_fwd(t.D, 64, 0, c->packed + c->off_wf, c->packed + c->off_bf, x, out, B, A, h, w, c->s, stream));
#undef RC
  return LFSR_OK;
}

static int distgssr_backward_impl(lfsr_distgssr* c, const float* x, const float* dout, int B, int h, int w, void* workspace, size_t workspace_bytes,
                                  float* grads, size_t n_grads, void* stream);

int lfsr_distgssr_backward(lfsr_distgssr* c, const float* x, const float* dout, int B, int h, int w, void* workspace, size_t workspace_bytes,
                           float* grads, size_t n_grads, void* stream) {
  const int rc = distgssr_backward_impl(c, x, dout, B, h, w, workspace, workspace_bytes, grads, n_grads, stream);
  if (rc != LFSR_OK && c && c->side) { (void)hipStreamSynchronize(c->side); (void)hipStreamSynchronize(lfsr_stream(stream)); }
  return rc;
}

static int distgssr_backward_impl(lfsr_distgssr* c, const float* x, const float* dout, int B, int h, int w, void* workspace, size_t workspace_bytes,
                                  float* grads, size_t n_grads, void* stream) {
  if (!c || !x || !dout || !workspace || !grads || B <= 0 || h <= 0 || w <= 0 || !c->finalized || n_grads != c->n_params) return LFSR_E_ARG;
  if (!(c->A & 1)) return LFSR_E_ARG;
  TrainWs t;
  train_layout(c, B, h, w, (float*)workspace, t);
  if (workspace_bytes < t.total * sizeof(float)) return LFSR_E_WS;
  const int A = c->A, AA = A * A, nimg = B * AA;
  const int npix = nimg * h * w;
  const float L = 0.1f;
  hipStream_t st = lfsr_stream(stream);
  int rc;
#define RC(call) do { rc = (call); if (rc) return rc; } while (0)
  auto G = [&](const std::string& k) -> float* { return grads + c->slots.at(k).grad_off; };
  bool overlap_br = false;
  {
    const char* osel = lfsr_sel("LFSR_BWD_OVERLAP");
    const int omode = osel ? atoi(osel) : 2;
    hipStreamCaptureStatus cs = hipStreamCaptureStatusNone;
    if (omode && hipStreamIsCapturing(st, &cs) == hipSuccess && cs == hipStreamCaptureStatusNone) {
      if (!c->side) {
        bool ok = hipStreamCreateWithFlags(&c->side, hipStreamNonBlocking) == hipSuccess;
        ok = ok && hipEventCreateWithFlags(&c->ev_fork, hipEventDisableTiming) == hipSuccess && hipEventCreateWithFlags(&c->ev_join, hipEventDisableTiming) == hipSuccess;
        ok = ok && hipEventCreateWithFlags(&c->ev_a, hipEventDisableTiming) == hipSuccess && hipEventCreateWithFlags(&c->ev_b, hipEventDisableTiming) == hipSuccess;
        if (!ok) { if (c->side) (void)hipStreamDestroy(c->side); c->side = nullptr; }
      }
      overlap_br = c->side != nullptr && (omode & 2);
    }
  }
  auto wgrad3 = [&](const std::string& key, const float* xin, const float* g, int g_stride) -> int {
    int r = lfsr_wgrad_conv3_launch(g, g_stride, 0, xin, 64, 0, t.P[0], nimg, h, w, st);
    if (!r) r = lfsr_wgrad_reduce(t.P[0], lfsr_wgrad_conv3_blocks(nimg, h, w), nullptr, 0, G(key), 64, 64, 9, 0, 0, 0, 0, 0, st);
    return r;
  };
  auto dgrad3 = [&](const float* dy, int dy_stride, const std::string& key, float* dx, const float* r1, const float* r2_unused, const float* mk, int mk_stride) -> int {
    (void)r2_unused;
    return lfsr_conv3x3_bwd_data(dy, dy_stride, 0, c->wT(key), dx, 64, 0, r1, 64, 0, mk, mk_stride, 0, L, nimg, h, w, st);
  };
  auto pick = [&](const float* a, const float* b, const float* d) -> float* {
    for (int i = 0; i < 4; ++i)
      if (t.g[i] != a && t.g[i] != b && t.g[i] != d) return t.g[i];
    return nullptr;
  };

  float* dD = t.g[0];
  RC(lfsr_head_bwd_data(dout, c->packed + c->off_wf, dD, t.G16, B, A, h, w, c->s, st));
  {
    float* dWf = t.small;
    float* colp = t.small + 16 * 64;
    RC(lfsr_wgrad_launch(LFSR_IN_SAME, LFSR_IN_SAME, t.G16, 16, 0, t.D, 64, 0, t.P[0], npix, 16, 64, 1, h, w, 1, st));
    RC(lfsr_wgrad_reduce(t.P[0], lfsr_wgrad_splits(npix, 1, 64), nullptr, 0, dWf, 16, 64, 1, 0, 0, 0, 0, 0, st));
    int nblk = 0;
    RC(lfsr_colsum(t.G16, npix, 16, colp, &nblk, st));
    if ((size_t)(16 * 64 + nblk * 16) > 64 * 1024) return LFSR_E_WS;
    RC(lfsr_head_fold_bwd(dWf, colp, nblk, c->w("upsample.0.weight"), c->w("upsample.0.bias"), c->w("upsample.2.weight"),
                          G("upsample.0.weight"), G("upsample.0.bias"), G("upsample.2.weight"), c->s, st));
  }
  const float* last = t.GOUT[c->G - 1];
  RC(wgrad3("disentg.conv.weight", last, dD, 64));
  float* gcur = pick(dD, nullptr, nullptr);
  RC(dgrad3(dD, 64, "disentg.conv.weight", gcur, nullptr, nullptr, nullptr, 0));
  for (int g = c->G - 1; g >= 0; --g) {
    float* dG = gcur;
    bool skip_fused = false;
    const float* blk_last = t.OUT[g * c->NB + c->NB - 1];
    std::string gk = "disentg.Group." + std::to_string(g) + ".conv.weight";
    RC(wgrad3(gk, blk_last, dG, 64));
    float* gy = pick(dD, dG, nullptr);
    RC(dgrad3(dG, 64, gk, gy, nullptr, nullptr, nullptr, 0));
    for (int b = c->NB - 1; b >= 0; --b) {
      const int i = g * c->NB + b;
      std::string p = "disentg.Group." + std::to_string(g) + ".Block." + std::to_string(b) + ".";
      const float* Xin = b > 0 ? t.OUT[i - 1] : (g > 0 ? t.GOUT[g - 1] : t.F0);
      float* gx = pick(dD, dG, gy);
      RC(wgrad3(p + "fuse.2.weight", t.FZ[i], gy, 64));
      RC(dgrad3(gy, 64, p + "fuse.2.weight", t.dF, nullptr, nullptr, t.FZ[i], 64));
      {
        float* Pw = t.PA;
        int rc5 = lfsr_wgrad_pw144_launch(t.dF, 64, 0, t.CAT[i], 144, 0, Pw, npix, st);
        int slabs = lfsr_wgrad_pw144_blocks(npix);
        if (rc5 == LFSR_E_ARG) {
          Pw = t.P[0];
          rc5 = lfsr_wgrad_launch(LFSR_IN_SAME, LFSR_IN_SAME, t.dF, 64, 0, t.CAT[i], 144, 0, Pw, npix, 64, 144, 1, h, w, 1, st); slabs = lfsr_wgrad_splits(npix, 1, 144);
        }
        RC(rc5);
        RC(lfsr_wgrad_reduce(Pw, slabs, nullptr, 0, G(p + "fuse.0.weight"), 64, 144, 1, 0, 0, 0, 0, 0, st));
      }
      {
        LfsrGemm q{};
        q.in_mode = LFSR_IN_SAME; q.out_mode = LFSR_OUT_SAME; q.cin = 64; q.X = t.dF; q.x_stride = 64; q.Wp = c->wT(p + "fuse.0.weight");
        q.Y = t.dCAT; q.y_stride = 144; q.Mk = t.CAT[i]; q.mk_stride = 144; q.mk_slope = L;
        q.M = npix; q.N = 144; q.A = 1; q.h = 1; q.w = 1; q.ntaps = 1; q.CH = 144;
        RC(lfsr_bwd_gemm(q, st));
      }
      RC(wgrad3(p + "SpaConv.2.weight", t.S1[i], t.dCAT, 144));
      RC(dgrad3(t.dCAT, 144, p + "SpaConv.2.weight", t.dS1, nullptr, nullptr, t.S1[i], 64));
      RC(wgrad3(p + "SpaConv.0.weight", Xin, t.dS1, 64));
      if (b == 0 && !skip_fused) {
        const int r2rc = lfsr_conv3x3_bwd_data_r2(t.dS1, 64, c->wT(p + "SpaConv.0.weight"), gx, gy, dG, nimg, h, w, st);
        if (r2rc == LFSR_OK) skip_fused = true; else if (r2rc != LFSR_E_ARG) return r2rc;
      }
      if (!(b == 0 && skip_fused)) RC(dgrad3(t.dS1, 64, p + "SpaConv.0.weight", gx, gy, nullptr, nullptr, 0));
      const float *wa0 = c->w(p + "AngConv.0.weight"), *wa0T = c->wT(p + "AngConv.0.weight"), *wa2T = c->wT(p + "AngConv.2.weight");
      const float *we0 = c->w(p + "EPIConv.0.weight"), *we0T = c->wT(p + "EPIConv.0.weight"), *we2T = c->wT(p + "EPIConv.2.weight");
      if (!overlap_br) {
        RC(lfsr_ang_branch_bwd(t.dCAT, 144, 64, Xin, t.A16[i], wa0, wa0T, wa2T, gx, G(p + "AngConv.0.weight"), G(p + "AngConv.2.weight"), t.dA16, t.PA, B, A, h, w, L, st));
        RC(lfsr_epi_branch_bwd(t.dCAT, 144, 80, 112, Xin, t.EH[i], t.EV[i], we0, we0T, we2T, gx, G(p + "EPIConv.0.weight"), G(p + "EPIConv.2.weight"), t.dE32, t.dE32V, t.P,
                               B, A, h, w, L, st));
      } else {
        if (hipEventRecord(c->ev_fork, st) != hipSuccess || hipStreamWaitEvent(c->side, c->ev_fork, 0) != hipSuccess) return LFSR_E_ARG;
        RC(lfsr_ang_branch_bwd_p1(t.dCAT, 144, 64, Xin, t.A16[i], wa2T, G(p + "AngConv.0.weight"), G(p + "AngConv.2.weight"), t.dA16, t.PA, B, A, h, w, L, c->side));
        if (hipEventRecord(c->ev_a, c->side) != hipSuccess) return LFSR_E_ARG;
        RC(lfsr_epi_branch_bwd_p1(t.dCAT, 144, 80, 112, t.EH[i], t.EV[i], we2T, G(p + "EPIConv.2.weight"), t.dE32, t.dE32V, t.P, B, A, h, w, L, st));
        if (hipEventRecord(c->ev_b, st) != hipSuccess || hipStreamWaitEvent(c->side, c->ev_b, 0) != hipSuccess) return LFSR_E_ARG;
        RC(lfsr_epi_branch_bwd_p2w(t.dE32, t.dE32V, Xin, G(p + "EPIConv.0.weight"), t.P, B, A, h, w, c->side));
        if (hipEventRecord(c->ev_join, c->side) != hipSuccess) return LFSR_E_ARG;
        if (hipStreamWaitEvent(st, c->ev_a, 0) != hipSuccess) return LFSR_E_ARG;
        RC(lfsr_ang_branch_bwd_p2(t.dA16, wa0, wa0T, gx, B, A, h, w, st));
        RC(lfsr_epi_branch_bwd_p2d(t.dE32, t.dE32V, we0, we0T, gx, B, A, h, w, st));
        if (hipStreamWaitEvent(st, c->ev_join, 0) != hipSuccess) return LFSR_E_ARG;
      }
      gy = gx;
    }
    if (!skip_fused) RC(lfsr_add_inplace(gy, dG, (long long)npix * 64, st));
    gcur = gy;
  }
  RC(lfsr_add_inplace(gcur, dD, (long long)npix * 64, st));
  RC(lfsr_init_gather9(x, t.XG9, B, A, h, w, st));
  RC(lfsr_wgrad_launch(LFSR_IN_SAME, LFSR_IN_SAME, gcur, 64, 0, t.XG9, 16, 0, t.P[0], npix, 64, 16, 1, h, w, 1, st));
  RC(lfsr_wgrad_reduce(t.P[0], lfsr_wgrad_splits(npix, 1, 16), nullptr, 0, G("init_conv.weight"), 64, 16, 1, 0, 0, 0, 9, 0, st));
#undef RC
  return LFSR_OK;
}

}
```

### ntire-2026-light-field-image-super-resolution-challenge---track-2-efficiency_amd/csrc/epi_b3.hip

```cpp
#include <stdlib.h>

#include "lfsr_internal.h"

#ifndef EB_VAR
#define EB_VAR 0
#endif
#ifndef EB_ABL
#define EB_ABL 0
#endif

namespace {

typedef float f32x4e __attribute__((ext_vector_type(4)));
typedef unsigned u32x4e __attribute__((ext_vector_type(4)));

constexpr int EB_LINES = 8;
constexpr int EB_STAGE_SLOTS = 5 * 3 * 4 * 32;
constexpr int EB_STAGE_BYTES = EB_STAGE_SLOTS * 16;
constexpr int EB_W2_SLOTS = 3 * 4 * 160;
constexpr int EB_W2_BYTES = EB_W2_SLOTS * 16;
constexpr int EB_SMEM = 4 * EB_STAGE_BYTES + EB_W2_BYTES;

struct EpiB3Args {
  const float* X; int x_stride; int x_choff; int x_bytes;
  const uint4* W1p;
  const uint4* W2p;
  float* Y; int y_stride; int choffH; int choffV; int y_bytes;
  float* TH; float* TV;
  int B, H, W;
  int tilesH, tilesV;
  int tpiH, tpiV;
  float slope;
};

__device__ __forceinline__ unsigned eb_hi_pair(unsigned hi_src, unsigned lo_src) { return __builtin_amdgcn_perm(hi_src, lo_src, 0x07060302u); }
__device__ __forceinline__ float eb_residual(float a) { return a - __uint_as_float(__float_as_uint(a) & 0xffff0000u); }

__device__ __forceinline__ void eb_split8(const f32x4e lo, const f32x4e hi, u32x4e& p0, u32x4e& p1, u32x4e& p2) {
  const float a[8] = {lo.x, lo.y, lo.z, lo.w, hi.x, hi.y, hi.z, hi.w};
#pragma unroll
  for (int j = 0; j < 4; ++j) { unsigned t0, t1, t2; lfsr_split_pair(a[2 * j], a[2 * j + 1], t0, t1, t2); p0[j] = t0; p1[j] = t1; p2[j] = t2; }
}

__device__ __forceinline__ void eb_mfma(f32x4e& c, const u32x4e a, const u32x4e b) {
  asm volatile("v_mfma_f32_16x16x32_bf16 %0, %1, %2, %0" : "+v"(c) : "v"(a), "v"(b));
}

__device__ __forceinline__ void eb_six2(f32x4e& c0, f32x4e& c1, const u32x4e a0, const u32x4e a1, const u32x4e a2,
                                        const u32x4e x00, const u32x4e x01, const u32x4e x02, const u32x4e x10, const u32x4e x11, const u32x4e x12) {
  eb_mfma(c0, a2, x00); eb_mfma(c1, a2, x10);
  eb_mfma(c0, a0, x02); eb_mfma(c1, a0, x12);
  eb_mfma(c0, a1, x01); eb_mfma(c1, a1, x11);
  eb_mfma(c0, a1, x00); eb_mfma(c1, a1, x10);
  eb_mfma(c0, a0, x01); eb_mfma(c1, a0, x11);
  eb_mfma(c0, a0, x00); eb_mfma(c1, a0, x10);
}

template <int CTRL>
__device__ __forceinline__ float eb_dpp0(float v) {
  return __builtin_bit_cast(float, __builtin_amdgcn_update_dpp(0, __builtin_bit_cast(int, v), CTRL, 0xf, 0xf, true));
}
template <int D>
__device__ __forceinline__ void eb_shift_add(f32x4e (&t)[2], const f32x4e (&z)[2]) {
  constexpr int SAME = D > 0 ? 0x100 + D : 0x110 - D;
  constexpr int WRAP = D > 0 ? 0x110 + (16 - D) : 0x100 + (16 + D);
#pragma unroll
  for (int r = 0; r < 4; ++r) {
    t[0][r] += eb_dpp0<SAME>(z[0][r]);
    t[1][r] += eb_dpp0<SAME>(z[1][r]);
    if (D > 0) t[0][r] += eb_dpp0<WRAP>(z[1][r]);
    else t[1][r] += eb_dpp0<WRAP>(z[0][r]);
  }
}

__global__ __launch_bounds__(512) void k_epi_b3(EpiB3Args p) {
  extern __shared__ __attribute__((aligned(16))) unsigned char smem_raw[];
  unsigned char* const sW = smem_raw;
  unsigned char* const sW2 = smem_raw + 4 * EB_STAGE_BYTES;
  constexpr int A = 5;
  constexpr int EOOB = (int)0x80000000u;
  const int tid = threadIdx.x, lane = tid & 63, wave = tid >> 6;
  const int l15 = lane & 15, g = lane >> 4;
  const int phase = __builtin_amdgcn_readfirstlane(wave >> 2);
  const int HW = p.H * p.W;
  const int ngroups = p.tilesH + p.tilesV;
  const int nb = (int)gridDim.x;
  const int vb = (nb & 7) ? (int)blockIdx.x : ((int)blockIdx.x & 7) * (nb >> 3) + ((int)blockIdx.x >> 3);

  const __amdgpu_buffer_rsrc_t rsX = __builtin_amdgcn_make_buffer_rsrc(const_cast<float*>(p.X), 0, p.x_bytes, 0x00020000);
  const __amdgpu_buffer_rsrc_t rsY = __builtin_amdgcn_make_buffer_rsrc(p.Y, 0, p.y_bytes, 0x00020000);

  struct Line { int vert, base, len, vstride, pstride, choff; long long rowbase; int rowstep; };
  const int nfr = ngroups / nb, nfull = nfr * nb, rem = ngroups - nfull;
  const int fsub = rem == 0 ? 1 : (rem * 4 <= nb ? 4 : rem * 2 <= nb ? 2 : 1);
  const int nunits = nfr + (vb < rem * fsub ? 1 : 0);
  auto line_of = [&](int it) -> Line {
    Line L;
    int grp, l0 = 0, nl = EB_LINES;
    if (it < nfr) grp = vb + it * nb;
    else if (it < nunits) { grp = nfull + vb / fsub; nl = EB_LINES / fsub; l0 = (vb % fsub) * nl; }
    else grp = ngroups;
    int tile;
    if (p.tpiH > 0) {
      const int per = p.tpiH + p.tpiV, item = grp / per, r = grp - item * per;
      L.vert = r >= p.tpiH;
      tile = L.vert ? item * p.tpiV + (r - p.tpiH) : item * p.tpiH + r;
    } else {
      L.vert = grp >= p.tilesH;
      tile = L.vert ? grp - p.tilesH : grp;
    }
    L.len = L.vert ? p.H : p.W;
    const int across = L.vert ? p.W : p.H;
    const int nlines = p.B * A * across;
    L.vstride = L.vert ? A * HW : HW;
    L.pstride = L.vert ? p.W : 1;
    L.choff = L.vert ? p.choffV : p.choffH;
    const int ln = tile * EB_LINES + l0 + wave;
    L.base = -1; L.rowbase = 0; L.rowstep = 0;
    if (grp < ngroups && wave < nl && ln < nlines) {
      const int q = ln / across, o = ln - q * across;
      if (!L.vert) L.base = q * A * HW + o * p.W;
      else { const int b = q / A, v = q - b * A; L.base = (b * A * A + v) * HW + o; }
      L.rowbase = L.vert ? (long long)q * p.H * p.W + o : ((long long)q * p.H + o) * p.W;
      L.rowstep = L.vert ? p.W : 1;
    }
    return L;
  };

  f32x4e rawA[2][2], rawB[2][2];
  u32x4e pA0[2], pA1[2], pA2[2], pB0[2], pB1[2], pB2[2];
  auto load_x = [&](const Line& L, int j, f32x4e (&xr)[2][2]) {
    const int vv = j >> 1, ks = j & 1;
    const int soff = (vv * L.vstride * p.x_stride + 32 * ks) * 4;
#pragma unroll
    for (int nt = 0; nt < 2; ++nt) {
      const int s = 16 * nt + l15;
      const int off = (L.base >= 0 && s < L.len) ? ((L.base + s * L.pstride) * p.x_stride + p.x_choff + 8 * g) * 4 : EOOB;
      xr[nt][0] = __builtin_bit_cast(f32x4e, __builtin_amdgcn_raw_buffer_load_b128(rsX, off, soff, 0));
      xr[nt][1] = __builtin_bit_cast(f32x4e, __builtin_amdgcn_raw_buffer_load_b128(rsX, off == EOOB ? EOOB : off + 16, soff, 0));
    }
  };
  uint4 wr[4];
  auto load_w = [&](int half_idx) {
    const uint4* src = p.W1p + half_idx * EB_STAGE_SLOTS;
#pragma unroll
    for (int i = 0; i < 4; ++i) {
      const int idx = tid + 512 * i;
      wr[i] = idx < EB_STAGE_SLOTS ? src[idx] : make_uint4(0u, 0u, 0u, 0u);
    }
  };
  auto store_w = [&](int buf, int ks) {
    uint4* dst = reinterpret_cast<uint4*>(sW + (buf * 2 + ks) * EB_STAGE_BYTES);
#pragma unroll
    for (int i = 0; i < 4; ++i) {
      const int idx = tid + 512 * i;
      if (idx < EB_STAGE_SLOTS) dst[idx] = wr[i];
    }
  };

  int it = 0;
  if (nunits == 0) return;
  Line L = line_of(0);
  load_x(L, 0, rawA);
  load_x(L, 1, rawB);
  load_w(0);
  {
    uint4 w2r[4];
#pragma unroll
    for (int i = 0; i < 4; ++i) { const int idx = tid + 512 * i; w2r[i] = idx < EB_W2_SLOTS ? p.W2p[idx] : make_uint4(0u, 0u, 0u, 0u); }
#pragma unroll
    for (int i = 0; i < 4; ++i) { const int idx = tid + 512 * i; if (idx < EB_W2_SLOTS) reinterpret_cast<uint4*>(sW2)[idx] = w2r[i]; }
  }
  store_w(0, 0);
  load_w(1);
  store_w(0, 1);
#pragma unroll
  for (int nt = 0; nt < 2; ++nt) eb_split8(rawA[nt][0], rawA[nt][1], pA0[nt], pA1[nt], pA2[nt]);
  __syncthreads();
  int cur = 0;
  const int aoff = (g * 32 + l15) * 16;
  const unsigned char* const w2b = sW2 + (g * 160 + l15) * 16;

  for (;;) {
    const bool more = it + 1 < nunits;
    const Line Ln = line_of(it + 1);
    f32x4e acc[5][2][2];
#pragma unroll
    for (int dx = 0; dx < 5; ++dx)
#pragma unroll
      for (int mt = 0; mt < 2; ++mt) { acc[dx][mt][0] = f32x4e{0.f, 0.f, 0.f, 0.f}; acc[dx][mt][1] = acc[dx][mt][0]; }
#pragma unroll
    for (int dx = 0; dx < 5; ++dx) asm volatile("s_nop 1" : "+v"(acc[dx][0][0]), "+v"(acc[dx][0][1]), "+v"(acc[dx][1][0]), "+v"(acc[dx][1][1]));

    auto step = [&](int j, u32x4e (&u0)[2], u32x4e (&u1)[2], u32x4e (&u2)[2], f32x4e (&rs)[2][2], u32x4e (&d0)[2], u32x4e (&d1)[2], u32x4e (&d2)[2],
                    f32x4e (&rd)[2][2]) {
      const int vv = j >> 1, ks = j & 1;
      if (!(EB_ABL & 8)) {
        if (j + 2 < 10) load_x(L, j + 2, rd);
        else load_x(Ln, j + 2 - 10, rd);
      }
      if (!(EB_ABL & 4)) load_w(2 * (vv + 1 < A ? vv + 1 : 0) + ks);
      asm volatile("s_nop 4" : "+v"(u0[0]), "+v"(u1[0]), "+v"(u2[0]), "+v"(u0[1]), "+v"(u1[1]), "+v"(u2[1]));
      const unsigned char* wb = sW + (cur * 2 + ks) * EB_STAGE_BYTES + aoff;
      u32x4e af[2][3];
      auto load_a = [&](int c, u32x4e (&a)[3]) {
        const int dx = c >> 1, mt = c & 1;
#pragma unroll
        for (int pl = 0; pl < 3; ++pl) a[pl] = *reinterpret_cast<const u32x4e*>(wb + ((dx * 3 + pl) * 128 + 16 * mt) * 16);
      };
      load_a(0, af[0]);
#pragma unroll
      for (int c = 0; c < 10; ++c) {
        const int dx = c >> 1, mt = c & 1;
        if (c + 1 < 10 && !(EB_ABL & 2)) load_a(c + 1, af[(c + 1) & 1]);
        constexpr int ABL2 = (EB_ABL & 2) ? 0 : 1;
        eb_six2(acc[dx][mt][0], acc[dx][mt][1], af[(c & 1) * ABL2][0], af[(c & 1) * ABL2][1], af[(c & 1) * ABL2][2], u0[0], u1[0], u2[0], u0[1], u1[1], u2[1]);
        if (!(EB_ABL & 1) && c == ((phase && !(EB_VAR & 4)) ? 5 : 0)) {
          asm volatile("" : "+v"(rs[0][0]), "+v"(rs[0][1]), "+v"(rs[1][0]), "+v"(rs[1][1]));
#pragma unroll
          for (int nt = 0; nt < 2; ++nt) eb_split8(rs[nt][0], rs[nt][1], d0[nt], d1[nt], d2[nt]);
          asm volatile("" : "+v"(d0[0]), "+v"(d1[0]), "+v"(d2[0]), "+v"(d0[1]), "+v"(d1[1]), "+v"(d2[1]));
        }
      }
      if (!(EB_ABL & 4)) store_w(cur ^ 1, ks);
      if (ks) { if (!(EB_ABL & 32)) __syncthreads(); cur ^= 1; }
    };
#pragma unroll 1
    for (int jj = 0; jj < 10; jj += 2) {
      step(jj, pA0, pA1, pA2, rawB, pB0, pB1, pB2, rawA);
      step(jj + 1, pB0, pB1, pB2, rawA, pA0, pA1, pA2, rawB);
    }

#pragma unroll
    for (int dx = 0; dx < 5; ++dx)
      asm volatile("s_nop 15\n\ts_nop 15" : "+v"(acc[dx][0][0]), "+v"(acc[dx][0][1]), "+v"(acc[dx][1][0]), "+v"(acc[dx][1][1]));
    if (EB_ABL & 16) {
      f32x4e sacc = acc[0][0][0];
#pragma unroll
      for (int dx = 0; dx < 5; ++dx) sacc += acc[dx][0][1] + acc[dx][1][0] + acc[dx][1][1] + acc[dx][0][0];
      if (L.base >= 0 && l15 < L.len) *reinterpret_cast<f32x4e*>(p.Y + (long long)(L.base + l15 * L.pstride) * p.y_stride + L.choff + 4 * g) = sacc;
      if (!more) break;
      ++it; L = Ln;
      continue;
    }
    f32x4e tv[2][2];
#pragma unroll
    for (int mt = 0; mt < 2; ++mt) {
      tv[mt][0] = acc[2][mt][0]; tv[mt][1] = acc[2][mt][1];
      eb_shift_add<-2>(tv[mt], acc[0][mt]);
      eb_shift_add<-1>(tv[mt], acc[1][mt]);
      eb_shift_add<1>(tv[mt], acc[3][mt]);
      eb_shift_add<2>(tv[mt], acc[4][mt]);
    }
    {
      float* tsave = L.vert ? p.TV : p.TH;
      const bool save = tsave && L.base >= 0;
#pragma unroll
      for (int mt = 0; mt < 2; ++mt)
#pragma unroll
        for (int nt = 0; nt < 2; ++nt) {
#pragma unroll
          for (int r = 0; r < 4; ++r) { const float v = tv[mt][nt][r]; tv[mt][nt][r] = (EB_VAR & 1) ? (v >= 0.f ? v : v * p.slope) : fmaxf(v, v * p.slope); }
          const int pos = 16 * nt + l15;
          if (save && pos < L.len) *reinterpret_cast<f32x4e*>(tsave + (L.rowbase + (long long)pos * L.rowstep) * 32 + 16 * mt + 4 * g) = tv[mt][nt];
        }
      if (save) asm volatile("s_nop 1" : "+v"(tv[0][0]), "+v"(tv[0][1]), "+v"(tv[1][0]), "+v"(tv[1][1]));
    }
    u32x4e t0[2], t1[2], t2[2];
#pragma unroll
    for (int nt = 0; nt < 2; ++nt) eb_split8(tv[0][nt], tv[1][nt], t0[nt], t1[nt], t2[nt]);
    asm volatile("s_nop 4" : "+v"(t0[0]), "+v"(t1[0]), "+v"(t2[0]), "+v"(t0[1]), "+v"(t1[1]), "+v"(t2[1]));
    int yoff[2];
#pragma unroll
    for (int nt = 0; nt < 2; ++nt) {
      const int pos = 16 * nt + l15;
      yoff[nt] = (L.base >= 0 && pos < L.len) ? ((L.base + pos * L.pstride) * p.y_stride + L.choff + 4 * g) * 4 : EOOB;
    }
    const int ychunk = L.vstride * p.y_stride * 4;
    u32x4e w2f[2][2][3];
    auto load_w2 = [&](int mp, u32x4e (&a)[2][3]) {
#pragma unroll
      for (int h = 0; h < 2; ++h)
#pragma unroll
        for (int pl = 0; pl < 3; ++pl) a[h][pl] = *reinterpret_cast<const u32x4e*>(w2b + ((pl * 4) * 160 + 16 * (2 * mp + h)) * 16);
    };
    load_w2(0, w2f[0]);
#pragma unroll
    for (int mp = 0; mp < 5; ++mp) {
      if (mp + 1 < 5) load_w2(mp + 1, w2f[(mp + 1) & 1]);
      f32x4e o[2][2];
#pragma unroll
      for (int h = 0; h < 2; ++h) { o[h][0] = f32x4e{0.f, 0.f, 0.f, 0.f}; o[h][1] = o[h][0]; }
      asm volatile("s_nop 1" : "+v"(o[0][0]), "+v"(o[0][1]), "+v"(o[1][0]), "+v"(o[1][1]));
#pragma unroll
      for (int h = 0; h < 2; ++h)
        eb_six2(o[h][0], o[h][1], w2f[mp & 1][h][0], w2f[mp & 1][h][1], w2f[mp & 1][h][2], t0[0], t1[0], t2[0], t0[1], t1[1], t2[1]);
      asm volatile("s_nop 15\n\ts_nop 15" : "+v"(o[0][0]), "+v"(o[0][1]), "+v"(o[1][0]), "+v"(o[1][1]));
#pragma unroll
      for (int nt = 0; nt < 2; ++nt)
#pragma unroll
        for (int h = 0; h < 2; ++h) {
          f32x4e v = o[h][nt];
#pragma unroll
          for (int r = 0; r < 4; ++r) v[r] = (EB_VAR & 1) ? (v[r] >= 0.f ? v[r] : v[r] * p.slope) : fmaxf(v[r], v[r] * p.slope);
          if (EB_VAR & 2) { if (yoff[nt] != EOOB) *reinterpret_cast<f32x4e*>(reinterpret_cast<char*>(p.Y) + (long long)yoff[nt] + (long long)mp * ychunk + 64 * h) = v; }
          else __builtin_amdgcn_raw_buffer_store_b128(__builtin_bit_cast(u32x4e, v), rsY, yoff[nt], __builtin_amdgcn_readfirstlane(mp * ychunk + 64 * h), 0);
          asm volatile("s_nop 1" : "+v"(v));
        }
    }
    if (!more) break;
    ++it;
    L = Ln;
  }
}

__device__ __forceinline__ void eb_planes8(const float* src, uint4& p0, uint4& p1, uint4& p2) {
  unsigned h0[8], h1[8], h2[8];
#pragma unroll
  for (int j = 0; j < 8; ++j) {
    const float a = src[j];
    const float r = eb_residual(a), q = eb_residual(r);
    h0[j] = __float_as_uint(a) >> 16; h1[j] = __float_as_uint(r) >> 16; h2[j] = __float_as_uint(q) >> 16;
  }
  p0 = make_uint4(h0[0] | (h0[1] << 16), h0[2] | (h0[3] << 16), h0[4] | (h0[5] << 16), h0[6] | (h0[7] << 16));
  p1 = make_uint4(h1[0] | (h1[1] << 16), h1[2] | (h1[3] << 16), h1[4] | (h1[5] << 16), h1[6] | (h1[7] << 16));
  p2 = make_uint4(h2[0] | (h2[1] << 16), h2[2] | (h2[3] << 16), h2[4] | (h2[5] << 16), h2[6] | (h2[7] << 16));
}

__device__ __forceinline__ void eb_pack_one(const float* __restrict__ src, uint4* __restrict__ dst, int kind, int i) {
  uint4 p0, p1, p2;
  if (kind == 0) {
    if (i >= 5 * 2 * 5 * 4 * 32) return;
    const int n = i & 31, g = (i >> 5) & 3, dx = (i >> 7) % 5, r = (i >> 7) / 5, ks = r & 1, v = r >> 1;
    eb_planes8(src + ((5 * dx + v) * 32 + n) * 64 + 32 * ks + 8 * g, p0, p1, p2);
    uint4* o = dst + (v * 2 + ks) * EB_STAGE_SLOTS + (dx * 3 * 4 + g) * 32 + n;
    o[0] = p0; o[4 * 32] = p1; o[8 * 32] = p2;
  } else {
    if (i >= 4 * 160) return;
    const int n = i % 160, g = i / 160;
    float kk[8];
#pragma unroll
    for (int jx = 0; jx < 8; ++jx) kk[jx] = src[n * 32 + 16 * (jx >> 2) + 4 * g + (jx & 3)];
    eb_planes8(kk, p0, p1, p2);
    uint4* o = dst + g * 160 + n;
    o[0] = p0; o[4 * 160] = p1; o[8 * 160] = p2;
  }
}

__global__ __launch_bounds__(256) void k_pack_epi_b3(const float* __restrict__ src, uint4* __restrict__ dst, int kind) {
  eb_pack_one(src, dst, kind, blockIdx.x * 256 + threadIdx.x);
}

__global__ __launch_bounds__(256) void k_pack_epi_b3_batch(const LfsrPackDesc* __restrict__ tab) {
  const LfsrPackDesc d = tab[blockIdx.y];
  eb_pack_one(d.src, reinterpret_cast<uint4*>(d.dst), d.kind, blockIdx.x * 256 + threadIdx.x);
}

}

int lfsr_pack_epi_b3(const float* direct_packed, float* out, int kind, hipStream_t st) {
  if (!direct_packed || !out || (kind != 0 && kind != 1) || ((uintptr_t)out & 15)) return LFSR_E_ARG;
  hipLaunchKernelGGL(k_pack_epi_b3, dim3(kind == 0 ? 25 : 3), dim3(256), 0, st, direct_packed, reinterpret_cast<uint4*>(out), kind);
  LFSR_CHECK_LAUNCH();
  return LFSR_OK;
}

int lfsr_pack_epi_b3_batch(const LfsrPackDesc* table_dev, int n, hipStream_t st) {
  if (!table_dev || n <= 0) return n == 0 ? LFSR_OK : LFSR_E_ARG;
  hipLaunchKernelGGL(k_pack_epi_b3_batch, dim3(25, (unsigned)n), dim3(256), 0, st, table_dev);
  LFSR_CHECK_LAUNCH();
  return LFSR_OK;
}

int lfsr_epi_b3_launch(const float* x, int x_stride, int x_choff, const float* w1_planes, const float* w2_planes, float* y, int y_stride,
                       int choffH, int choffV, float* t_h, float* t_v, int B, int A, int h, int w, int which, float slope, hipStream_t st) {
  if (A != 5 || h > 32 || w > 32 || h <= 0 || w <= 0 || B <= 0) return LFSR_E_ARG;
  if ((x_stride | x_choff | y_stride | choffH | choffV) & 3) return LFSR_E_ARG;
  if (((uintptr_t)x | (uintptr_t)y | (uintptr_t)w1_planes | (uintptr_t)w2_planes | (uintptr_t)t_h | (uintptr_t)t_v) & 15) return LFSR_E_ARG;
  if ((long long)B * A * A * h * w * x_stride * 4 >= (1LL << 31) || (long long)B * A * A * h * w * y_stride * 4 >= (1LL << 31)) return LFSR_E_ARG;
  if (!(slope >= 0.f && slope <= 1.f)) return LFSR_E_ARG;
  static std::atomic<bool> attr_set[64];
  static std::atomic<int> cus[64];
  int dev = 0;
  if (hipGetDevice(&dev) != hipSuccess || dev < 0 || dev >= 64) return LFSR_E_ARG;
  if (!attr_set[dev]) {
    hipError_t e = hipFuncSetAttribute(reinterpret_cast<const void*>(k_epi_b3), hipFuncAttributeMaxDynamicSharedMemorySize, EB_SMEM);
    if (e != hipSuccess) return LFSR_HIP_ERR(e);
    int v = 0;
    cus[dev] = (hipDeviceGetAttribute(&v, hipDeviceAttributeMultiprocessorCount, dev) == hipSuccess && v > 0) ? v : 256;
    attr_set[dev] = true;
  }
  EpiB3Args p{};
  p.X = x; p.x_stride = x_stride; p.x_choff = x_choff; p.x_bytes = (int)((long long)B * A * A * h * w * x_stride * 4);
  p.W1p = reinterpret_cast<const uint4*>(w1_planes); p.W2p = reinterpret_cast<const uint4*>(w2_planes);
  p.Y = y; p.y_stride = y_stride; p.choffH = choffH; p.choffV = choffV; p.TH = t_h; p.TV = t_v;
  p.y_bytes = (int)((long long)B * A * A * h * w * y_stride * 4);
  p.B = B; p.H = h; p.W = w; p.slope = slope;
  p.tilesH = (which & 1) ? (B * A * h + EB_LINES - 1) / EB_LINES : 0;
  p.tilesV = (which & 2) ? (B * A * w + EB_LINES - 1) / EB_LINES : 0;
  const int ngroups = p.tilesH + p.tilesV;
  if (ngroups <= 0) return LFSR_E_ARG;
  if (which == 3 && (A * h) % EB_LINES == 0 && (A * w) % EB_LINES == 0) { p.tpiH = A * h / EB_LINES; p.tpiV = A * w / EB_LINES; }
  int grid = cus[dev];
  if (grid > ngroups) grid = ngroups;
  hipLaunchKernelGGL(k_epi_b3, dim3((unsigned)grid), dim3(512), EB_SMEM, st, p);
  LFSR_CHECK_LAUNCH();
  return LFSR_OK;
}
```

### ntire-2026-light-field-image-super-resolution-challenge---track-2-efficiency_amd/csrc/lfsr_internal.h

```cpp
#pragma once
#include "lfsr_common.h"

enum { LFSR_IN_SAME = 0, LFSR_IN_CONV3 = 1, LFSR_IN_ANG = 2, LFSR_IN_EPIH = 3, LFSR_IN_EPIV = 4,
       LFSR_IN_CHK_H = 5, LFSR_IN_CHK_V = 6, LFSR_IN_LINE_H = 7, LFSR_IN_LINE_V = 8 };
enum { LFSR_OUT_SAME = 0, LFSR_OUT_VIEWS = 1, LFSR_OUT_EPIH = 2, LFSR_OUT_EPIV = 3 };

#if defined(__HIPCC__)
#ifndef LFSR_SPLIT_DOT2
#define LFSR_SPLIT_DOT2 1
#endif
__device__ __forceinline__ void lfsr_split_pair(float a0, float a1, unsigned& p0, unsigned& p1, unsigned& p2) {
  typedef __bf16 lfsr_bf16x2 __attribute__((ext_vector_type(2)));
  p0 = __builtin_amdgcn_perm(__float_as_uint(a1), __float_as_uint(a0), 0x07060302u);
#if LFSR_SPLIT_DOT2
  unsigned klo, khi;
  asm("s_mov_b32 %0, 0xbf80" : "=s"(klo));
  asm("s_mov_b32 %0, 0xbf800000" : "=s"(khi));
  const float r0 = __builtin_amdgcn_fdot2_f32_bf16(__builtin_bit_cast(lfsr_bf16x2, p0), __builtin_bit_cast(lfsr_bf16x2, klo), a0, false);
  const float r1 = __builtin_amdgcn_fdot2_f32_bf16(__builtin_bit_cast(lfsr_bf16x2, p0), __builtin_bit_cast(lfsr_bf16x2, khi), a1, false);
  p1 = __builtin_amdgcn_perm(__float_as_uint(r1), __float_as_uint(r0), 0x07060302u);
  const float q0 = __builtin_amdgcn_fdot2_f32_bf16(__builtin_bit_cast(lfsr_bf16x2, p1), __builtin_bit_cast(lfsr_bf16x2, klo), r0, false);
  const float q1 = __builtin_amdgcn_fdot2_f32_bf16(__builtin_bit_cast(lfsr_bf16x2, p1), __builtin_bit_cast(lfsr_bf16x2, khi), r1, false);
#else
  const float r0 = a0 - __uint_as_float(__float_as_uint(a0) & 0xffff0000u), r1 = a1 - __uint_as_float(__float_as_uint(a1) & 0xffff0000u);
  p1 = __builtin_amdgcn_perm(__float_as_uint(r1), __float_as_uint(r0), 0x07060302u);
  const float q0 = r0 - __uint_as_float(__float_as_uint(r0) & 0xffff0000u), q1 = r1 - __uint_as_float(__float_as_uint(r1) & 0xffff0000u);
#endif
  p2 = __builtin_amdgcn_perm(__float_as_uint(q1), __float_as_uint(q0), 0x07060302u);
}
#endif

#ifdef LFSR_CONV_DIAG
extern float* g_lfsr_diag_buf;
extern "C" int lfsr_diag_set_buffer(float* buf);
#endif

struct LfsrOpTimer {
  LfsrOpTimer(const char* op, int a, int b, hipStream_t st);
  ~LfsrOpTimer();
  LfsrOpTimer(const LfsrOpTimer&) = delete;
  LfsrOpTimer& operator=(const LfsrOpTimer&) = delete;
 private:
  int slot_, gen_;
  hipStream_t st_;
};

int lfsr_conv3x3_halo_launch(const float* x, int x_stride, int x_choff, const float* w_packed, float* y, int y_stride, int y_choff,
                             const float* r1, int r1_stride, int r1_choff, const float* r2, int r2_stride, int r2_choff,
                             const float* mk, int mk_stride, int mk_choff, float mk_slope,
                             int n_img, int h, int w, float slope, hipStream_t st);
int lfsr_conv3x3_halo_tail_launch(const float* x, int x_stride, int x_choff, const float* w_packed, float* y, int y_stride, int y_choff,
                                  const float* r1, int r1_stride, int r1_choff, const float* r2, int r2_stride, int r2_choff,
                                  const float* mk, int mk_stride, int mk_choff, float mk_slope,
                                  int n_img, int h, int w, float slope, int tile_begin, int tile_count, hipStream_t st);
#define LFSR_CONV3_DIRECT_FLOATS (9 * 64 * 64)
#define LFSR_CONV3_WINO2_FLOATS (16 * 64 * 64)
#define LFSR_CONV3_WINO4_FLOATS (36 * 64 * 64)
#define LFSR_CONV3_WINO_FLOATS (LFSR_CONV3_WINO2_FLOATS + LFSR_CONV3_WINO4_FLOATS)
int lfsr_pack_wino(const float* direct_packed, float* out, hipStream_t st);
enum { LFSR_W_WINO2 = 1, LFSR_W_WINO4 = 2, LFSR_W_ALL = 3 };
int lfsr_conv3_variant_mask();
const char* lfsr_conv3_fwd_sel();
const char* lfsr_conv3_dgrad_sel();
struct LfsrPackDesc { const float* src; float* dst; float* dst2; int kind, O, C, T, Npad, perm, ch, flip; };
int lfsr_pack_generic_batch(const LfsrPackDesc* table_dev, int n, hipStream_t st);
int lfsr_pack_conv3_raw_wino4_batch(const LfsrPackDesc* table_dev, int n, hipStream_t st);
int lfsr_pack_epi_wino_batch(const LfsrPackDesc* table_dev, int n, hipStream_t st);
int lfsr_pack_conv3_raw_wino4(const float* w_raw, float* direct_out, float* wino4_out, int transposed, hipStream_t st);
int lfsr_pack_wino_m(const float* direct_packed, float* out, int mask, hipStream_t st);
int lfsr_pack_conv_weight_m(const float* w, float* packed, int O, int C, int taps, int perm, int ch, int mask, void* stream);
int lfsr_pack_weight_T_m(const float* w, float* out, int O, int C, int T, int flip, int mask, hipStream_t st);
int lfsr_pack_wino4(const float* direct_packed, float* out, hipStream_t st);
int lfsr_conv3x3_wino4_launch(const float* x, int x_stride, int x_choff, const float* w_wino4, float* y, int y_stride, int y_choff,
                              const float* r1, int r1_stride, int r1_choff, const float* r2, int r2_stride, int r2_choff,
                              const float* mk, int mk_stride, int mk_choff, float mk_slope,
                              int n_img, int h, int w, float slope, hipStream_t st);
int lfsr_conv3x3_wino_launch(const float* x, int x_stride, int x_choff, const float* w_wino, const float* w_direct, float* y, int y_stride, int y_choff,
                             const float* r1, int r1_stride, int r1_choff, const float* r2, int r2_stride, int r2_choff,
                             const float* mk, int mk_stride, int mk_choff, float mk_slope,
                             int n_img, int h, int w, float slope, const char* sel, hipStream_t st);
bool lfsr_ang_fused_ok(int A);
int lfsr_ang_fused_launch(const float* x, int x_stride, int x_choff, const float* w1_packed, const float* w2_packed, float* t, float* y,
                          int y_stride, int y_choff, int B, int A, int h, int w, float slope, hipStream_t st);
#define LFSR_EPI_WINO_FLOATS (5 * 6 * 32 * 64)
#define LFSR_EPI_B3_W1_FLOATS (25 * 32 * 64 * 3 / 2)
#define LFSR_EPI_B3_W2_FLOATS (160 * 32 * 3 / 2)
bool lfsr_epi_use_b3();
int lfsr_pack_epi_b3(const float* direct_packed, float* out, int kind, hipStream_t st);
int lfsr_pack_epi_b3_batch(const LfsrPackDesc* table_dev, int n, hipStream_t st);
int lfsr_epi_b3_launch(const float* x, int x_stride, int x_choff, const float* w1_planes, const float* w2_planes, float* y, int y_stride,
                       int choffH, int choffV, float* t_h, float* t_v, int B, int A, int h, int w, int which, float slope, hipStream_t st);
int lfsr_pack_epi_wino(const float* w1_direct_packed, float* out, hipStream_t st);
bool lfsr_epi_fused_ok(int A, int h, int w);
int lfsr_epi_fused_launch(const float* x, int x_stride, int x_choff, const float* w1_packed, const float* w2_packed, float* y, int y_stride,
                          int choffH, int choffV, float* t_h, float* t_v, int B, int A, int h, int w, int which, float slope, hipStream_t st);

extern "C" int lfsr_epiconv_gather(const float* x, int x_stride, int x_choff, const float* w1_packed, const float* w2_packed,
                        float* tmp, float* y, int y_stride, int y_choff, int B, int A, int h, int w, int vertical, float slope, hipStream_t st);

struct LfsrGemm {
  int in_mode, out_mode, cin;
  const float* X; int x_stride, x_choff;
  const float* Wp;
  float* Y; int y_stride, y_choff;
  const float* R1; int r1_stride, r1_choff;
  const float* Mk; int mk_stride, mk_choff; float mk_slope;
  int M, N, A, h, w, ntaps, CH;
};
int lfsr_bwd_gemm(const LfsrGemm& g, hipStream_t st);
int lfsr_conv3x3_bwd_data_r2(const float* dy, int dy_stride, const float* wT_packed, float* dx, const float* r1, const float* r2, int n_img, int h, int w, hipStream_t st);
int lfsr_conv3x3_bwd_data(const float* dy, int dy_stride, int dy_choff, const float* wT_packed, float* dx, int dx_stride, int dx_choff,
                          const float* r1, int r1_stride, int r1_choff, const float* mk, int mk_stride, int mk_choff, float mk_slope,
                          int n_img, int h, int w, hipStream_t st);
int lfsr_head_bwd_data(const float* dout, const float* wf, float* df, float* g16, int B, int A, int h, int w, int s, hipStream_t st);
int lfsr_colsum(const float* g, int M, int N, float* partial, int* nblk_out, hipStream_t st);
int lfsr_head_fold_bwd(const float* dWf, const float* colsum_partial, int nblk, const float* w0, const float* b0, const float* w2,
                       float* dw0, float* db0, float* dw2, int s, hipStream_t st);
int lfsr_init_gather9(const float* x, float* xg, int B, int A, int h, int w, hipStream_t st);
int lfsr_add_inplace(float* a, const float* b, long long n, hipStream_t st);
int lfsr_pack_weight_chunkT(const float* w, float* out, int O, int C, int ch, int perm, hipStream_t st);

int lfsr_rowgemm_dgrad144_launch(const float* dy, int dy_stride, int dy_choff, const float* wT_packed, const float* mk, int mk_stride, int mk_choff, float mk_slope,
                                 float* dx, int dx_stride, int dx_choff, long long M, hipStream_t st);
int lfsr_rowgemm_ln_launch(const float* x, int x_stride, int x_choff, int K, const float* w_packed, const float* ln_g, const float* ln_b, float ln_eps, int ln_cols,
                           const float* pe, int pe_stride, int pe_rows, int pe_div, float* y, int y_stride, int y_choff,
                           float* y2, int y2_stride, int y2_choff, int split_n, long long M, int N, hipStream_t st);
int lfsr_rowgemm_b3_ln_launch(const float* x, int x_stride, int x_choff, int K, const float* w_packed, const float* ln_g, const float* ln_b, float ln_eps, int ln_cols,
                              const float* pe, int pe_stride, int pe_rows, int pe_div, float* y, int y_stride, int y_choff,
                              float* y2, int y2_stride, int y2_choff, int split_n, long long M, int N, hipStream_t st);
int lfsr_lnlin_b3_launch(const float* x, int x_stride, int x_choff, int K, const float* w_packed, const float* ln_g, const float* ln_b, float ln_eps, int ln_cols,
                         const float* pe, int pe_stride, int pe_rows, int pe_div, float* y, int y_stride, int y_choff,
                         float* y2, int y2_stride, int y2_choff, int split_n, long long M, int N, hipStream_t st);
int lfsr_rowgemm_b3_dgrad_launch(const float* dy, int dy_stride, int dy_choff, const float* wT_packed, const float* mk, int mk_stride, int mk_choff, float mk_slope,
                                 float* dx, int dx_stride, int dx_choff, long long M, int N, hipStream_t st);
int lfsr_rowgemm_b3_launch(const float* x, int x_stride, int x_choff, int K, const float* w_packed, const float* res, int res_stride, int res_choff,
                           float* y, int y_stride, int y_choff, long long M, int N, float slope, hipStream_t st);
int lfsr_rowgemm_launch(const float* x, int x_stride, int x_choff, int K, const float* w_packed, const float* bias,
                        const float* res, int res_stride, int res_choff, float* y, int y_stride, int y_choff, long long M, int N, float slope, hipStream_t st);

int lfsr_ffn_ln_launch(const float* x, int x_stride, int x_choff, const float* ln_g, const float* ln_b, float ln_eps, const float* w1_packed, const float* w2_packed,
                       const float* res, int res_stride, int res_choff, float* y, int y_stride, int y_choff,
                       long long M, int K1, int H, int N2, float slope, hipStream_t st, const void* wsplit = nullptr);

int lfsr_ffn_b3_launch(const float* x, int x_stride, int x_choff, const float* ln_g, const float* ln_b, float ln_eps, const float* w1_packed, const float* w2_packed,
                       const float* res, int res_stride, int res_choff, float* y, int y_stride, int y_choff,
                       long long M, int K1, int H, int N2, float slope, hipStream_t st, const void* wsplit = nullptr);
size_t lfsr_ffn_b3_presplit_bytes(int K1, int H, int N2);
int lfsr_ffn_b3_presplit(const float* w1_packed, const float* w2_packed, int K1, int H, int N2, void* out, hipStream_t st);

int lfsr_epi_attn_mfma_launch(const float* q, int q_stride, int q_choff, const float* k, int k_stride, int k_choff, const float* v, int v_stride, int v_choff,
                              float* o, int o_stride, int o_choff, int nheads, int ns0, int ns1, int ns2, long long bs0, long long bs1, long long bs2,
                              int n1, int n2, long long st1, long long st2, int l1, int r1, int l2, int r2, int clip2, hipStream_t st);
int lfsr_win_attn_mfma_launch(const float* q, int q_stride, int q_choff, const float* k, int k_stride, int k_choff, const float* v, int v_stride, int v_choff,
                              float* o, int o_stride, int o_choff, int nheads, int ns0, int ns1, int ns2, long long bs0, long long bs1, long long bs2,
                              int n1, int n2, long long st1, long long st2, int l1, int r1, int l2, int r2, int clip2, hipStream_t st);

int lfsr_wgrad_splits(int M, int ntaps, int K);
size_t lfsr_wgrad_partial_floats(int M, int ntaps, int N, int K);
int lfsr_wgrad_launch(int gmode, int xmode, const float* G, int g_stride, int g_choff, const float* X, int x_stride, int x_choff,
                      float* P, int M, int N, int K, int A, int h, int w, int ntaps, hipStream_t st);
int lfsr_wgrad_conv3_blocks(int n_img, int h, int w);
int lfsr_wgrad_pw144_blocks(int M);
int lfsr_wgrad_pw144_launch(const float* G, int g_stride, int g_choff, const float* X, int x_stride, int x_choff, float* P, int M, hipStream_t st);
int lfsr_wgrad_epi0_blocks(int B, int A, int h, int w, int vert);
int lfsr_ang0_dgrad_launch(const float* dA16, const float* w_direct, float* dx, int dx_stride, int dx_choff, int B, int A, int h, int w, hipStream_t st);
int lfsr_epi0_dgrad_launch(const float* dE, const float* w_direct, float* dx, int dx_stride, int dx_choff, int B, int A, int h, int w, int vert, hipStream_t st);
int lfsr_wgrad_epi0_launch(const float* dE, const float* dE_v, const float* X, int x_stride, int x_choff, float* P, int B, int A, int h, int w, int vert, hipStream_t st);
int lfsr_wgrad_conv3_launch(const float* G, int g_stride, int g_choff, const float* X, int x_stride, int x_choff, float* P,
                            int n_img, int h, int w, hipStream_t st);
int lfsr_wgrad_reduce(const float* P, int nsplit, const float* P2, int nsplit2, float* dW, int O, int C, int T, int perm, int ch,
                      int accumulate, int c_valid, int chunk_mode, hipStream_t st);
int lfsr_pack_weight_T(const float* w, float* out, int O, int C, int T, int flip, hipStream_t st);

size_t lfsr_branch_bwd_partial_floats(int B, int A, int h, int w);
int lfsr_ang_branch_bwd(const float* dcat, int dc_stride, int dc_choff, const float* xin, const float* a16, const float* w0_packed, const float* w0T_packed,
                        const float* w2T_packed, float* dx, float* dw0, float* dw2, float* dA16, float* P, int B, int A, int h, int w, float slope, hipStream_t st);
int lfsr_epi_branch_bwd(const float* dcat, int dc_stride, int choff_h, int choff_v, const float* xin, const float* eh, const float* ev,
                        const float* w0_packed, const float* w0T_packed, const float* w2T_packed, float* dx, float* dw0, float* dw2,
                        float* dEh, float* dEv, float* const P[4], int B, int A, int h, int w, float slope, hipStream_t st);
int lfsr_ang_branch_bwd_p1(const float* dcat, int dc_stride, int dc_choff, const float* xin, const float* a16, const float* w2T_packed, float* dw0, float* dw2,
                           float* dA16, float* P, int B, int A, int h, int w, float slope, hipStream_t st);
int lfsr_ang_branch_bwd_p2(const float* dA16, const float* w0_packed, const float* w0T_packed, float* dx, int B, int A, int h, int w, hipStream_t st);
int lfsr_epi_branch_bwd_p1(const float* dcat, int dc_stride, int choff_h, int choff_v, const float* eh, const float* ev, const float* w2T_packed, float* dw2,
                           float* dEh, float* dEv, float* const P[4], int B, int A, int h, int w, float slope, hipStream_t st);
int lfsr_epi_branch_bwd_p2d(const float* dEh, const float* dEv, const float* w0_packed, const float* w0T_packed, float* dx, int B, int A, int h, int w, hipStream_t st);
int lfsr_epi_branch_bwd_p2w(const float* dEh, const float* dEv, const float* xin, float* dw0, float* const P[4], int B, int A, int h, int w, hipStream_t st);
```

Before: 2005.

## Fuse angular/EPI second stages with fuse.0 into one branch-tail kernel

Adds a distg_tail kernel that, per 16-pixel tile, computes the angular stage-2 and EPI H/V stage-2 convolutions on the fly from their stage-1 intermediates. It concatenates the results with the spatial branch in per-wave LDS and applies the fuse.0 1x1 conv using split-bf16 MFMA. The angular and EPI stage-1 kernels gain template variants that skip stage 2 and write only intermediates. This removes the 144-channel CAT buffer round trip and separate stage-2 passes, at the cost of more LDS use, complex hand-scheduled code and recomputation of EPI stage-2 per view.

New measurement: 2136, median of 6. 1.07x the previous value.

```diff
diff --git a/include/lfsr_hip.h b/include/lfsr_hip.h
--- a/include/lfsr_hip.h
+++ b/include/lfsr_hip.h
@@ -57,6 +57,11 @@
 int lfsr_epiconv_hv_fwd(const float* x, int x_stride, int x_choff, const float* w1_packed, const float* w2_packed,
                         float* tmp, float* y, int y_stride, int choff_h, int choff_v, int B, int A, int h, int w,
                         float slope, void* stream);
+
+int lfsr_distg_branch_tail_fwd(const float* x, int x_stride, int x_choff, const float* spa, int spa_stride, int spa_choff,
+                               const float* w_ang0, const float* w_ang2, const float* w_epi0, const float* w_epi2, const float* w_fuse0,
+                               float* t_a, float* t_h, float* t_v, float* y, int y_stride, int y_choff, int B, int A, int h, int w, float slope,
+                               void* stream);
 
 int lfsr_initconv_fwd(const float* x, const float* w, float* y, int y_stride, int y_choff, int B, int A, int h, int wd,
                       void* stream);
diff --git a/ntire-2026-light-field-image-super-resolution-challenge---track-2-efficiency_amd/capi.py b/ntire-2026-light-field-image-super-resolution-challenge---track-2-efficiency_amd/capi.py
--- a/ntire-2026-light-field-image-super-resolution-challenge---track-2-efficiency_amd/capi.py
+++ b/ntire-2026-light-field-image-super-resolution-challenge---track-2-efficiency_amd/capi.py
@@ -31,6 +31,7 @@
     "lfsr_angconv_fwd": (c_i, [c_p, c_i, c_i, c_p, c_p, c_p, c_p, c_i, c_i, c_i, c_i, c_i, c_i, c_f, c_p]),
     "lfsr_epiconv_fwd": (c_i, [c_p, c_i, c_i, c_p, c_p, c_p, c_p, c_i, c_i, c_i, c_i, c_i, c_i, c_i, c_f, c_p]),
     "lfsr_epiconv_hv_fwd": (c_i, [c_p, c_i, c_i, c_p, c_p, c_p, c_p, c_i, c_i, c_i, c_i, c_i, c_i, c_i, c_f, c_p]),
+    "lfsr_distg_branch_tail_fwd": (c_i, [c_p, c_i, c_i, c_p, c_i, c_i, c_p, c_p, c_p, c_p, c_p, c_p, c_p, c_p, c_p, c_i, c_i, c_i, c_i, c_i, c_i, c_f, c_p]),
     "lfsr_initconv_fwd": (c_i, [c_p, c_p, c_p, c_i, c_i, c_i, c_i, c_i, c_i, c_p]),
     "lfsr_fold_head": (c_i, [c_p, c_p, c_p, c_p, c_p, c_i, c_i, c_p]),
     "lfsr_upsample_head_fwd": (c_i, [c_p, c_i, c_i, c_p, c_p, c_p, c_p, c_i, c_i, c_i, c_i, c_i, c_p]),
@@ -552,6 +553,18 @@
     return out
 
 
+def distg_branch_tail(x, spa, w_ang0, w_ang2, w_epi0, w_epi2, w_fuse0, B, A, h, w, slope):
+    lib = load()
+    y = torch.empty((x.shape[0], 64), dtype=torch.float32, device=x.device)
+    t_a = torch.empty((B * h * w, 16), dtype=torch.float32, device=x.device)
+    t_h = torch.empty((B * A * h * w, 32), dtype=torch.float32, device=x.device)
+    t_v = torch.empty((B * A * h * w, 32), dtype=torch.float32, device=x.device)
+    check(lib.lfsr_distg_branch_tail_fwd(dev_ptr(x), x.shape[1], 0, dev_ptr(spa), spa.shape[1], 0, dev_ptr(w_ang0), dev_ptr(w_ang2), dev_ptr(w_epi0),
+                                         dev_ptr(w_epi2), dev_ptr(w_fuse0), dev_ptr(t_a), dev_ptr(t_h), dev_ptr(t_v), dev_ptr(y), 64, 0, B, A, h, w, slope,
+                                         stream_ptr()), "distg_branch_tail_fwd")
+    return y, t_a, t_h, t_v
+
+
 def initconv(x, w, A):
     lib = load()
     B, _, Hh, Ww = x.shape
diff --git a/ntire-2026-light-field-image-super-resolution-challenge---track-2-efficiency_amd/csrc/ang_fused.hip b/ntire-2026-light-field-image-super-resolution-challenge---track-2-efficiency_amd/csrc/ang_fused.hip
--- a/ntire-2026-light-field-image-super-resolution-challenge---track-2-efficiency_amd/csrc/ang_fused.hip
+++ b/ntire-2026-light-field-image-super-resolution-challenge---track-2-efficiency_amd/csrc/ang_fused.hip
@@ -17,6 +17,7 @@
   float slope;
 };
 
+template <bool S2>
 __global__ __launch_bounds__(512) void k_ang_fused(AngArgs p) {
   extern __shared__ __attribute__((aligned(16))) float sm[];
   const int AA = p.A * p.A, HW = p.H * p.W, M = p.B * HW;
@@ -52,7 +53,7 @@
 #pragma unroll
     for (int q = 0; q < 4; ++q) {
       const int idx = tid + q * 512;
-      w2v[q] = idx < AA * 64 ? reinterpret_cast<const float4*>(p.W2)[idx] : make_float4(0.f, 0.f, 0.f, 0.f);
+      w2v[q] = S2 && idx < AA * 64 ? reinterpret_cast<const float4*>(p.W2)[idx] : make_float4(0.f, 0.f, 0.f, 0.f);
     }
     if (g0 < ngroups) load_row(g0, 0, fb[0]);
 #pragma unroll
@@ -63,7 +64,7 @@
 #pragma unroll
     for (int q = 0; q < 4; ++q) {
       const int idx = tid + q * 512;
-      if (idx < AA * 64) reinterpret_cast<float4*>(sW2)[idx] = w2v[q];
+      if (S2 && idx < AA * 64) reinterpret_cast<float4*>(sW2)[idx] = w2v[q];
     }
   }
   __syncthreads();
@@ -109,6 +110,7 @@
     const float4 a2 = *reinterpret_cast<const float4*>(st + i * TROW + 4 * kq);
     if (ok) *reinterpret_cast<float4*>(p.T + (long long)m * 16 + 4 * kq) = a2;
     __builtin_amdgcn_wave_barrier();
+    if (!S2) continue;
     for (int view = 0; view < AA; ++view) {
       const float4 b = *reinterpret_cast<const float4*>(b2 + view * 256);
       f32x4a o = {0.f, 0.f, 0.f, 0.f};
@@ -141,12 +143,13 @@
 
 int lfsr_ang_fused_launch(const float* x, int x_stride, int x_choff, const float* w1_packed, const float* w2_packed, float* t, float* y,
                           int y_stride, int y_choff, int B, int A, int h, int w, float slope, hipStream_t st) {
-  if (!lfsr_ang_fused_ok(A)) return LFSR_E_ARG;
+  if (!lfsr_ang_fused_ok(A) || !t) return LFSR_E_ARG;
   static std::atomic<bool> attr_set[64];
   int dev = 0;
   if (hipGetDevice(&dev) != hipSuccess || dev < 0 || dev >= 64) return LFSR_E_ARG;
   if (!attr_set[dev]) {
-    hipError_t e = hipFuncSetAttribute(reinterpret_cast<const void*>(k_ang_fused), hipFuncAttributeMaxDynamicSharedMemorySize, 160 * 1024);
+    hipError_t e = hipFuncSetAttribute(reinterpret_cast<const void*>(k_ang_fused<true>), hipFuncAttributeMaxDynamicSharedMemorySize, 160 * 1024);
+    if (e == hipSuccess) e = hipFuncSetAttribute(reinterpret_cast<const void*>(k_ang_fused<false>), hipFuncAttributeMaxDynamicSharedMemorySize, 160 * 1024);
     if (e != hipSuccess) return LFSR_HIP_ERR(e);
     attr_set[dev] = true;
   }
@@ -157,7 +160,8 @@
   const int waves = 8;
   long long grid = (ngroups + waves - 1) / waves;
   if (grid > 256) grid = 256;
-  hipLaunchKernelGGL(k_ang_fused, dim3((unsigned)grid), dim3(waves * 64), lfsr_ang_fused_smem(A, waves), st, p);
+  if (y) hipLaunchKernelGGL(k_ang_fused<true>, dim3((unsigned)grid), dim3(waves * 64), lfsr_ang_fused_smem(A, waves), st, p);
+  else hipLaunchKernelGGL(k_ang_fused<false>, dim3((unsigned)grid), dim3(waves * 64), lfsr_ang_fused_smem(A, waves), st, p);
   LFSR_CHECK_LAUNCH();
   return LFSR_OK;
 }
diff --git a/ntire-2026-light-field-image-super-resolution-challenge---track-2-efficiency_amd/csrc/distg_tail.hip b/ntire-2026-light-field-image-super-resolution-challenge---track-2-efficiency_amd/csrc/distg_tail.hip
--- /dev/null
+++ b/ntire-2026-light-field-image-super-resolution-challenge---track-2-efficiency_amd/csrc/distg_tail.hip
@@ -0,0 +1,287 @@
+#include "lfsr_internal.h"
+
+namespace {
+
+typedef float f32x4t __attribute__((ext_vector_type(4)));
+typedef unsigned u32x4t __attribute__((ext_vector_type(4)));
+
+constexpr int DT_WAVES = 8;
+constexpr int DT_FPLANE = 64 * 160;
+constexpr int DT_FBYTES = 3 * DT_FPLANE * 2;
+constexpr int DT_ESLOTS = 3 * 4 * 160;
+constexpr int DT_EBYTES = DT_ESLOTS * 16;
+constexpr int DT_AFLOATS = 25 * 16 * 16;
+constexpr int DT_ABYTES = DT_AFLOATS * 4;
+constexpr int DT_CROW = 84;
+constexpr int DT_CBYTES = DT_WAVES * 16 * DT_CROW * 4;
+constexpr int DT_SMEM = DT_FBYTES + DT_EBYTES + DT_ABYTES + DT_CBYTES;
+
+struct DistgTailArgs {
+  const float* S; int s_stride; int s_choff; int s_bytes;
+  const float* TA; int ta_bytes;
+  const float* TH; const float* TV; int te_bytes;
+  const float* WA2;
+  const uint4* WE2p;
+  const float* WF;
+  float* Y; int y_stride; int y_choff; int y_bytes;
+  int B, H, W;
+  float slope;
+};
+
+__device__ __forceinline__ void dt_split8(const f32x4t lo, const f32x4t hi, u32x4t& p0, u32x4t& p1, u32x4t& p2) {
+  const float a[8] = {lo.x, lo.y, lo.z, lo.w, hi.x, hi.y, hi.z, hi.w};
+#pragma unroll
+  for (int j = 0; j < 4; ++j) { unsigned t0, t1, t2; lfsr_split_pair(a[2 * j], a[2 * j + 1], t0, t1, t2); p0[j] = t0; p1[j] = t1; p2[j] = t2; }
+}
+
+__device__ __forceinline__ void dt_mfma(f32x4t& c, const u32x4t a, const u32x4t b) {
+  asm volatile("v_mfma_f32_16x16x32_bf16 %0, %1, %2, %0" : "+v"(c) : "v"(a), "v"(b));
+}
+
+__device__ __forceinline__ void dt_six2(f32x4t& c0, const u32x4t (&a)[3], const u32x4t (&x)[3], f32x4t& c1, const u32x4t (&b)[3], const u32x4t (&y)[3]) {
+  dt_mfma(c0, a[2], x[0]); dt_mfma(c1, b[2], y[0]);
+  dt_mfma(c0, a[0], x[2]); dt_mfma(c1, b[0], y[2]);
+  dt_mfma(c0, a[1], x[1]); dt_mfma(c1, b[1], y[1]);
+  dt_mfma(c0, a[1], x[0]); dt_mfma(c1, b[1], y[0]);
+  dt_mfma(c0, a[0], x[1]); dt_mfma(c1, b[0], y[1]);
+  dt_mfma(c0, a[0], x[0]); dt_mfma(c1, b[0], y[0]);
+}
+
+__global__ __launch_bounds__(512) void k_distg_tail(DistgTailArgs p) {
+  extern __shared__ __attribute__((aligned(16))) unsigned char smem_raw[];
+  unsigned short* const sF = reinterpret_cast<unsigned short*>(smem_raw);
+  unsigned char* const sE = smem_raw + DT_FBYTES;
+  float* const sA = reinterpret_cast<float*>(smem_raw + DT_FBYTES + DT_EBYTES);
+  float* const sC = reinterpret_cast<float*>(smem_raw + DT_FBYTES + DT_EBYTES + DT_ABYTES);
+  constexpr int A = 5, AA = 25;
+  constexpr int EOOB = (int)0x80000000u;
+  const int tid = threadIdx.x, lane = tid & 63, wave = tid >> 6;
+  const int l15 = lane & 15, g = lane >> 4;
+  const int HW = p.H * p.W, M = p.B * HW;
+  const int ntiles = (M + 15) / 16;
+
+  for (int i = tid; i < 64 * 20; i += 512) {
+    const int r = i / 20, c = i - r * 20;
+    const bool ok = c * 8 < 144;
+    const float* src = p.WF + r * 144 + (ok ? c * 8 : 0);
+    f32x4t lo = *reinterpret_cast<const f32x4t*>(src), hi = *reinterpret_cast<const f32x4t*>(src + 4);
+    if (!ok) { lo = f32x4t{0.f, 0.f, 0.f, 0.f}; hi = lo; }
+    u32x4t w0, w1, w2;
+    dt_split8(lo, hi, w0, w1, w2);
+    const int slot = (c * 64 + r) * 8;
+    *reinterpret_cast<u32x4t*>(sF + 0 * DT_FPLANE + slot) = w0;
+    *reinterpret_cast<u32x4t*>(sF + 1 * DT_FPLANE + slot) = w1;
+    *reinterpret_cast<u32x4t*>(sF + 2 * DT_FPLANE + slot) = w2;
+  }
+  for (int i = tid; i < DT_ESLOTS; i += 512) reinterpret_cast<uint4*>(sE)[i] = p.WE2p[i];
+  for (int i = tid; i < DT_AFLOATS / 4; i += 512) reinterpret_cast<float4*>(sA)[i] = reinterpret_cast<const float4*>(p.WA2)[i];
+  __syncthreads();
+
+  const __amdgpu_buffer_rsrc_t rsS = __builtin_amdgcn_make_buffer_rsrc(const_cast<float*>(p.S), 0, p.s_bytes, 0x00020000);
+  const __amdgpu_buffer_rsrc_t rsA = __builtin_amdgcn_make_buffer_rsrc(const_cast<float*>(p.TA), 0, p.ta_bytes, 0x00020000);
+  const __amdgpu_buffer_rsrc_t rsH = __builtin_amdgcn_make_buffer_rsrc(const_cast<float*>(p.TH), 0, p.te_bytes, 0x00020000);
+  const __amdgpu_buffer_rsrc_t rsV = __builtin_amdgcn_make_buffer_rsrc(const_cast<float*>(p.TV), 0, p.te_bytes, 0x00020000);
+  const __amdgpu_buffer_rsrc_t rsY = __builtin_amdgcn_make_buffer_rsrc(p.Y, 0, p.y_bytes, 0x00020000);
+  float* const st = sC + wave * 16 * DT_CROW;
+  const unsigned char* const wE = sE + (g * 160 + l15) * 16;
+  const unsigned short* const wF = sF + (g * 64 + l15) * 8;
+  const float* const bA = sA + l15 * 16 + 4 * g;
+
+  for (int tile = (int)blockIdx.x * DT_WAVES + wave; tile < ntiles; tile += (int)gridDim.x * DT_WAVES) {
+    const int m = tile * 16 + l15;
+    const bool ok = m < M;
+    const int mb = ok ? m / HW : 0, myx = ok ? m - mb * HW : 0;
+    auto tro = [&](int q) { return ok ? (((mb * A + q) * HW + myx) * 32 + 4 * g) * 4 : EOOB; };
+    auto pixo = [&](int view) { return ok ? ((mb * AA + view) * HW + myx) : -1; };
+    const f32x4t a2 = __builtin_bit_cast(f32x4t, __builtin_amdgcn_raw_buffer_load_b128(rsA, ok ? (m * 16 + 4 * g) * 4 : EOOB, 0, 0));
+
+    f32x4t sr0[2][2], sr1[2][2], vr0[2], vr1[2], hr[2];
+    auto load_view = [&](int view, f32x4t (&sr)[2][2], f32x4t (&vr)[2]) {
+      const int pix = pixo(view);
+      const int so = pix >= 0 ? (pix * p.s_stride + p.s_choff + 8 * g) * 4 : EOOB;
+#pragma unroll
+      for (int s = 0; s < 2; ++s)
+#pragma unroll
+        for (int e = 0; e < 2; ++e) sr[s][e] = __builtin_bit_cast(f32x4t, __builtin_amdgcn_raw_buffer_load_b128(rsS, so == EOOB ? EOOB : so + (32 * s + 4 * e) * 4, 0, 0));
+      const int vo = tro(view % A);
+      vr[0] = __builtin_bit_cast(f32x4t, __builtin_amdgcn_raw_buffer_load_b128(rsV, vo, 0, 0));
+      vr[1] = __builtin_bit_cast(f32x4t, __builtin_amdgcn_raw_buffer_load_b128(rsV, vo == EOOB ? EOOB : vo + 64, 0, 0));
+    };
+    auto load_h = [&](int u) {
+      const int ho = tro(u);
+      hr[0] = __builtin_bit_cast(f32x4t, __builtin_amdgcn_raw_buffer_load_b128(rsH, ho, 0, 0));
+      hr[1] = __builtin_bit_cast(f32x4t, __builtin_amdgcn_raw_buffer_load_b128(rsH, ho == EOOB ? EOOB : ho + 64, 0, 0));
+    };
+    load_h(0);
+    load_view(0, sr0, vr0);
+    u32x4t hp[3];
+
+    auto body = [&](int view, f32x4t (&sr)[2][2], f32x4t (&vr)[2], f32x4t (&srn)[2][2], f32x4t (&vrn)[2]) {
+      const int u = view / A, v = view - A * u;
+      if (view + 1 < AA) load_view(view + 1, srn, vrn);
+      if (v == 0) dt_split8(hr[0], hr[1], hp[0], hp[1], hp[2]);
+      if (v == A - 1 && u + 1 < A) load_h(u + 1);
+
+      {
+        const float4 b = *reinterpret_cast<const float4*>(bA + view * 256);
+        f32x4t o = {0.f, 0.f, 0.f, 0.f};
+        o = __builtin_amdgcn_mfma_f32_16x16x4f32(a2.x, b.x, o, 0, 0, 0);
+        o = __builtin_amdgcn_mfma_f32_16x16x4f32(a2.y, b.y, o, 0, 0, 0);
+        o = __builtin_amdgcn_mfma_f32_16x16x4f32(a2.z, b.z, o, 0, 0, 0);
+        o = __builtin_amdgcn_mfma_f32_16x16x4f32(a2.w, b.w, o, 0, 0, 0);
+#pragma unroll
+        for (int r = 0; r < 4; ++r) {
+          float z = o[r];
+          z = z >= 0.f ? z : z * p.slope;
+          st[(4 * g + r) * DT_CROW + l15] = z;
+        }
+      }
+
+      {
+        u32x4t vp[3];
+        dt_split8(vr[0], vr[1], vp[0], vp[1], vp[2]);
+        asm volatile("s_nop 4" : "+v"(hp[0]), "+v"(hp[1]), "+v"(hp[2]), "+v"(vp[0]), "+v"(vp[1]), "+v"(vp[2]));
+        f32x4t e[2][2];
+#pragma unroll
+        for (int i = 0; i < 2; ++i) { e[i][0] = f32x4t{0.f, 0.f, 0.f, 0.f}; e[i][1] = e[i][0]; }
+        asm volatile("s_nop 1" : "+v"(e[0][0]), "+v"(e[0][1]), "+v"(e[1][0]), "+v"(e[1][1]));
+#pragma unroll
+        for (int h = 0; h < 2; ++h) {
+          u32x4t aH[3], aV[3];
+#pragma unroll
+          for (int pl = 0; pl < 3; ++pl) {
+            aH[pl] = *reinterpret_cast<const u32x4t*>(wE + ((pl * 4) * 160 + 16 * (2 * v + h)) * 16);
+            aV[pl] = *reinterpret_cast<const u32x4t*>(wE + ((pl * 4) * 160 + 16 * (2 * u + h)) * 16);
+          }
+          dt_six2(e[0][h], aH, hp, e[1][h], aV, vp);
+        }
+        asm volatile("s_nop 15\n\ts_nop 15" : "+v"(e[0][0]), "+v"(e[0][1]), "+v"(e[1][0]), "+v"(e[1][1]));
+#pragma unroll
+        for (int i = 0; i < 2; ++i)
+#pragma unroll
+          for (int h = 0; h < 2; ++h) {
+            f32x4t z = e[i][h];
+#pragma unroll
+            for (int r = 0; r < 4; ++r) z[r] = fmaxf(z[r], z[r] * p.slope);
+            *reinterpret_cast<f32x4t*>(st + l15 * DT_CROW + 16 + 32 * i + 16 * h + 4 * g) = z;
+          }
+      }
+      __builtin_amdgcn_wave_barrier();
+
+      u32x4t x0[5], x1[5], x2[5];
+#pragma unroll
+      for (int s = 0; s < 2; ++s) dt_split8(sr[s][0], sr[s][1], x0[s], x1[s], x2[s]);
+#pragma unroll
+      for (int s = 2; s < 5; ++s) {
+        const float* cp = st + l15 * DT_CROW + 32 * (s - 2) + 8 * g;
+        f32x4t lo = *reinterpret_cast<const f32x4t*>(cp), hi = *reinterpret_cast<const f32x4t*>(cp + 4);
+        if (s == 4 && g >= 2) { lo = f32x4t{0.f, 0.f, 0.f, 0.f}; hi = lo; }
+        dt_split8(lo, hi, x0[s], x1[s], x2[s]);
+      }
+      __builtin_amdgcn_wave_barrier();
+      f32x4t acc[4];
+#pragma unroll
+      for (int t = 0; t < 4; ++t) acc[t] = f32x4t{0.f, 0.f, 0.f, 0.f};
+#pragma unroll
+      for (int s = 0; s < 5; ++s) asm volatile("s_nop 4" : "+v"(x0[s]), "+v"(x1[s]), "+v"(x2[s]));
+      asm volatile("s_nop 1" : "+v"(acc[0]), "+v"(acc[1]), "+v"(acc[2]), "+v"(acc[3]));
+#pragma unroll
+      for (int s = 0; s < 5; ++s) {
+        const u32x4t xs[3] = {x0[s], x1[s], x2[s]};
+#pragma unroll
+        for (int t = 0; t < 4; t += 2) {
+          u32x4t wa[3], wb[3];
+#pragma unroll
+          for (int pl = 0; pl < 3; ++pl) {
+            wa[pl] = *reinterpret_cast<const u32x4t*>(wF + pl * DT_FPLANE + (4 * s * 64 + t * 16) * 8);
+            wb[pl] = *reinterpret_cast<const u32x4t*>(wF + pl * DT_FPLANE + (4 * s * 64 + (t + 1) * 16) * 8);
+          }
+          dt_six2(acc[t], wa, xs, acc[t + 1], wb, xs);
+        }
+      }
+      asm volatile("s_nop 15\n\ts_nop 15" : "+v"(acc[0]), "+v"(acc[1]), "+v"(acc[2]), "+v"(acc[3]));
+      const int pix = pixo(view);
+      const int yo = pix >= 0 ? (pix * p.y_stride + p.y_choff + 4 * g) * 4 : EOOB;
+#pragma unroll
+      for (int t = 0; t < 4; ++t) {
+        f32x4t z = acc[t];
+#pragma unroll
+        for (int r = 0; r < 4; ++r) z[r] = z[r] >= 0.f ? z[r] : z[r] * p.slope;
+        __builtin_amdgcn_raw_buffer_store_b128(__builtin_bit_cast(u32x4t, z), rsY, yo == EOOB ? EOOB : yo + 64 * t, 0, 0);
+        asm volatile("s_nop 1" : "+v"(z));
+      }
+    };
+#pragma unroll 1
+    for (int view = 0; view < AA - 1; view += 2) {
+      body(view, sr0, vr0, sr1, vr1);
+      body(view + 1, sr1, vr1, sr0, vr0);
+    }
+    body(AA - 1, sr0, vr0, sr1, vr1);
+  }
+}
+
+}
+
+int lfsr_distg_tail_launch(const float* spa, int spa_stride, int spa_choff, const float* t_a, const float* t_h, const float* t_v, const float* wa2_packed,
+                           const float* we2_planes, const float* wf_packed, float* y, int y_stride, int y_choff, int B, int A, int h, int w, float slope,
+                           hipStream_t st) {
+  if (A != 5 || B <= 0 || h <= 0 || w <= 0 || !spa || !t_a || !t_h || !t_v || !wa2_packed || !we2_planes || !wf_packed || !y) return LFSR_E_ARG;
+  if ((spa_stride | spa_choff | y_stride | y_choff) & 3 || spa_stride < spa_choff + 64 || y_stride < y_choff + 64) return LFSR_E_ARG;
+  if (((uintptr_t)spa | (uintptr_t)t_a | (uintptr_t)t_h | (uintptr_t)t_v | (uintptr_t)wa2_packed | (uintptr_t)we2_planes | (uintptr_t)wf_packed | (uintptr_t)y) & 15)
+    return LFSR_E_ARG;
+  if (!(slope >= 0.f && slope <= 1.f)) return LFSR_E_ARG;
+  const long long npix = (long long)B * A * A * h * w;
+  if (npix * spa_stride * 4 >= (1LL << 31) || npix * y_stride * 4 >= (1LL << 31) || (long long)B * A * h * w * 32 * 4 >= (1LL << 31)) return LFSR_E_ARG;
+  static std::atomic<bool> attr_set[64];
+  static std::atomic<int> cus[64];
+  int dev = 0;
+  if (hipGetDevice(&dev) != hipSuccess || dev < 0 || dev >= 64) return LFSR_E_ARG;
+  if (!attr_set[dev]) {
+    hipError_t e = hipFuncSetAttribute(reinterpret_cast<const void*>(k_distg_tail), hipFuncAttributeMaxDynamicSharedMemorySize, DT_SMEM);
+    if (e != hipSuccess) return LFSR_HIP_ERR(e);
+    int v = 0;
+    cus[dev] = (hipDeviceGetAttribute(&v, hipDeviceAttributeMultiprocessorCount, dev) == hipSuccess && v > 0) ? v : 256;
+    attr_set[dev] = true;
+  }
+  DistgTailArgs p{};
+  p.S = spa; p.s_stride = spa_stride; p.s_choff = spa_choff; p.s_bytes = (int)(npix * spa_stride * 4);
+  p.TA = t_a; p.ta_bytes = (int)((long long)B * h * w * 16 * 4);
+  p.TH = t_h; p.TV = t_v; p.te_bytes = (int)((long long)B * A * h * w * 32 * 4);
+  p.WA2 = wa2_packed; p.WE2p = reinterpret_cast<const uint4*>(we2_planes); p.WF = wf_packed;
+  p.Y = y; p.y_stride = y_stride; p.y_choff = y_choff; p.y_bytes = (int)(npix * y_stride * 4);
+  p.B = B; p.H = h; p.W = w; p.slope = slope;
+  const long long ntiles = ((long long)B * h * w + 15) / 16;
+  long long grid = (ntiles + DT_WAVES - 1) / DT_WAVES;
+  if (grid > cus[dev]) grid = cus[dev];
+  hipLaunchKernelGGL(k_distg_tail, dim3((unsigned)grid), dim3(DT_WAVES * 64), DT_SMEM, st, p);
+  LFSR_CHECK_LAUNCH();
+  return LFSR_OK;
+}
+
+bool lfsr_distg_tail_ok(int A, int h, int w, const float* x, int x_stride, int x_choff, const float* t_h, const float* t_v) {
+  if (A != 5 || h <= 0 || w <= 0 || h > 32 || w > 32 || !lfsr_ang_fused_ok(A) || !lfsr_epi_use_b3()) return false;
+  const char* rsel = lfsr_sel("LFSR_ROWGEMM");
+  const char* asel = lfsr_sel("LFSR_ANG");
+  if ((rsel && (rsel[0] == 'f' || rsel[0] == '1')) || lfsr_sel("LFSR_NO_ROWGEMM") || (asel && asel[0] == 'g')) return false;
+  if ((x_stride | x_choff) & 3 || x_stride < x_choff + 64 || (((uintptr_t)x | (uintptr_t)t_h | (uintptr_t)t_v) & 15)) return false;
+  return true;
+}
+
+extern "C" int lfsr_distg_branch_tail_fwd(const float* x, int x_stride, int x_choff, const float* spa, int spa_stride, int spa_choff,
+                                          const float* w_ang0, const float* w_ang2, const float* w_epi0, const float* w_epi2, const float* w_fuse0,
+                                          float* t_a, float* t_h, float* t_v, float* y, int y_stride, int y_choff, int B, int A, int h, int w, float slope,
+                                          void* stream) {
+  LfsrOpTimer op_t("distg_tail", B, h * w, lfsr_stream(stream));
+  if (!x || !spa || !w_ang0 || !w_ang2 || !w_epi0 || !w_epi2 || !w_fuse0 || !t_a || !t_h || !t_v || !y || B <= 0) return LFSR_E_ARG;
+  if (!lfsr_distg_tail_ok(A, h, w, x, x_stride, x_choff, t_h, t_v)) return LFSR_E_ARG;
+  if ((spa_stride | spa_choff | y_stride | y_choff) & 3 || spa_stride < spa_choff + 64 || y_stride < y_choff + 64) return LFSR_E_ARG;
+  if (((uintptr_t)spa | (uintptr_t)t_a | (uintptr_t)w_ang2 | (uintptr_t)w_epi0 | (uintptr_t)w_epi2 | (uintptr_t)w_fuse0 | (uintptr_t)y) & 15) return LFSR_E_ARG;
+  if (!(slope >= 0.f && slope <= 1.f)) return LFSR_E_ARG;
+  const long long npix = (long long)B * A * A * h * w;
+  if (npix * x_stride * 4 >= (1LL << 31) || npix * spa_stride * 4 >= (1LL << 31) || npix * y_stride * 4 >= (1LL << 31)) return LFSR_E_ARG;
+  hipStream_t st = lfsr_stream(stream);
+  int rc = lfsr_ang_fused_launch(x, x_stride, x_choff, w_ang0, nullptr, t_a, nullptr, 0, 0, B, A, h, w, slope, st);
+  if (!rc) rc = lfsr_epi_b3_launch(x, x_stride, x_choff, w_epi0 + 25 * 32 * 64 + LFSR_EPI_WINO_FLOATS, nullptr, nullptr, 0, 0, 0, t_h, t_v, B, A, h, w, 3, slope, st);
+  if (!rc) rc = lfsr_distg_tail_launch(spa, spa_stride, spa_choff, t_a, t_h, t_v, w_ang2, w_epi2 + 160 * 32, w_fuse0, y, y_stride, y_choff, B, A, h, w, slope, st);
+  return rc;
+}
diff --git a/ntire-2026-light-field-image-super-resolution-challenge---track-2-efficiency_amd/csrc/distgssr.cpp b/ntire-2026-light-field-image-super-resolution-challenge---track-2-efficiency_amd/csrc/distgssr.cpp
--- a/ntire-2026-light-field-image-super-resolution-challenge---track-2-efficiency_amd/csrc/distgssr.cpp
+++ b/ntire-2026-light-field-image-super-resolution-challenge---track-2-efficiency_amd/csrc/distgssr.cpp
@@ -239,19 +239,20 @@
   return LFSR_OK;
 }
 
-static void ws_layout(const lfsr_distgssr* c, int B, int h, int w, size_t off[8], size_t* total) {
+static void ws_layout(const lfsr_distgssr* c, int B, int h, int w, size_t off[9], size_t* total) {
   const size_t npix = (size_t)B * c->A * c->A * h * w;
   size_t o = 0;
   for (int i = 0; i < 5; ++i) { off[i] = o; o += align64(npix * 64); }
   off[5] = o; o += align64(npix * 144);
   off[6] = o; o += align64((size_t)B * h * w * 16);
   off[7] = o; o += align64((size_t)B * c->A * h * w * 32);
+  off[8] = o; o += align64((size_t)B * c->A * h * w * 32);
   *total = o;
 }
 
 size_t lfsr_distgssr_workspace_bytes(const lfsr_distgssr* c, int B, int h, int w) {
   if (!c || B <= 0 || h <= 0 || w <= 0) return 0;
-  size_t off[8], tot;
+  size_t off[9], tot;
   ws_layout(c, B, h, w, off, &tot);
   return tot * sizeof(float);
 }
@@ -260,7 +261,7 @@
                                size_t workspace_bytes, float* const* taps, void* stream) {
   if (!c || !x || !out || !workspace || B <= 0 || h <= 0 || w <= 0 || !c->finalized) return LFSR_E_ARG;
   if ((uintptr_t)workspace & 15) return LFSR_E_ARG;
-  size_t off[8], tot;
+  size_t off[9], tot;
   ws_layout(c, B, h, w, off, &tot);
   if (workspace_bytes < tot * sizeof(float)) return LFSR_E_WS;
   if ((long long)B * c->A * c->A * h * w * 160 * 4 >= (1LL << 30)) return LFSR_E_ARG;
@@ -270,8 +271,11 @@
   float* CAT = ws + off[5];
   float* A16 = ws + off[6];
   float* E32 = ws + off[7];
+  float* EV32 = ws + off[8];
   const int A = c->A, AA = A * A, nimg = B * AA;
   const float L = 0.1f;
+  const char* tsel = lfsr_sel("LFSR_DISTG_TAIL");
+  const bool tail_ok = !(tsel && tsel[0] == '0') && (long long)nimg * h * w >= 2048 && lfsr_distg_tail_ok(A, h, w, nullptr, 64, 0, E32, EV32);
   int rc;
 #define RC(call) do { rc = (call); if (rc) return rc; } while (0)
 #define PROF(cls, call)                                                              \
@@ -310,6 +314,19 @@
       std::string p = "disentg.Group." + std::to_string(g) + ".Block." + std::to_string(b) + ".";
       float* o = pick(F0, gin, cur);
       PROF(0, conv(cur, p + "SpaConv.0.weight", T, 64, 0, nullptr, L));
+      if (tail_ok && !(taps && taps[4] && g == 0 && b == 0)) {
+        PROF(0, conv(T, p + "SpaConv.2.weight", o, 64, 0, nullptr, L));
+        hipStream_t st = lfsr_stream(stream);
+        PROF(1, lfsr_ang_fused_launch(cur, 64, 0, c->w(p + "AngConv.0.weight"), nullptr, A16, nullptr, 0, 0, B, A, h, w, L, st));
+        PROF(2, lfsr_epi_b3_launch(cur, 64, 0, c->w(p + "EPIConv.0.weight") + 25 * 32 * 64 + LFSR_EPI_WINO_FLOATS, nullptr, nullptr, 0, 0, 0, E32, EV32,
+                                   B, A, h, w, 3, L, st));
+        PROF(3, lfsr_distg_tail_launch(o, 64, 0, A16, E32, EV32, c->w(p + "AngConv.2.weight"), c->w(p + "EPIConv.2.weight") + 160 * 32,
+                                       c->w(p + "fuse.0.weight"), T, 64, 0, B, A, h, w, L, st));
+        PROF(0, conv(T, p + "fuse.2.weight", o, 64, 0, cur, 1.0f));
+        cur = o;
+        if (g == 0 && b == 0) RC(tap(1, cur, 64, 64));
+        continue;
+      }
       PROF(0, conv(T, p + "SpaConv.2.weight", CAT, 144, 0, nullptr, L));
       PROF(1, lfsr_angconv_fwd(cur, 64, 0, c->w(p + "AngConv.0.weight"), c->w(p + "AngConv.2.weight"), A16, CAT, 144, 64, B, A, h, w, L, stream));
       PROF(2, lfsr_epiconv_hv_fwd(cur, 64, 0, c->w(p + "EPIConv.0.weight"), c->w(p + "EPIConv.2.weight"), E32, CAT, 144, 80, 112, B, A, h, w, L, stream));
diff --git a/ntire-2026-light-field-image-super-resolution-challenge---track-2-efficiency_amd/csrc/epi_b3.hip b/ntire-2026-light-field-image-super-resolution-challenge---track-2-efficiency_amd/csrc/epi_b3.hip
--- a/ntire-2026-light-field-image-super-resolution-challenge---track-2-efficiency_amd/csrc/epi_b3.hip
+++ b/ntire-2026-light-field-image-super-resolution-challenge---track-2-efficiency_amd/csrc/epi_b3.hip
@@ -20,6 +20,7 @@
 constexpr int EB_W2_SLOTS = 3 * 4 * 160;
 constexpr int EB_W2_BYTES = EB_W2_SLOTS * 16;
 constexpr int EB_SMEM = 4 * EB_STAGE_BYTES + EB_W2_BYTES;
+constexpr int EB_SMEM1 = 4 * EB_STAGE_BYTES;
 
 struct EpiB3Args {
   const float* X; int x_stride; int x_choff; int x_bytes;
@@ -73,6 +74,7 @@
   }
 }
 
+template <bool S2>
 __global__ __launch_bounds__(512) void k_epi_b3(EpiB3Args p) {
   extern __shared__ __attribute__((aligned(16))) unsigned char smem_raw[];
   unsigned char* const sW = smem_raw;
@@ -164,7 +166,7 @@
   load_x(L, 0, rawA);
   load_x(L, 1, rawB);
   load_w(0);
-  {
+  if (S2) {
     uint4 w2r[4];
 #pragma unroll
     for (int i = 0; i < 4; ++i) { const int idx = tid + 512 * i; w2r[i] = idx < EB_W2_SLOTS ? p.W2p[idx] : make_uint4(0u, 0u, 0u, 0u); }
@@ -266,6 +268,12 @@
         }
       if (save) asm volatile("s_nop 1" : "+v"(tv[0][0]), "+v"(tv[0][1]), "+v"(tv[1][0]), "+v"(tv[1][1]));
     }
+    if (!S2) {
+      if (!more) break;
+      ++it;
+      L = Ln;
+      continue;
+    }
     u32x4e t0[2], t1[2], t2[2];
 #pragma unroll
     for (int nt = 0; nt < 2; ++nt) eb_split8(tv[0][nt], tv[1][nt], t0[nt], t1[nt], t2[nt]);
@@ -375,16 +383,18 @@
 int lfsr_epi_b3_launch(const float* x, int x_stride, int x_choff, const float* w1_planes, const float* w2_planes, float* y, int y_stride,
                        int choffH, int choffV, float* t_h, float* t_v, int B, int A, int h, int w, int which, float slope, hipStream_t st) {
   if (A != 5 || h > 32 || w > 32 || h <= 0 || w <= 0 || B <= 0) return LFSR_E_ARG;
+  if (!y && (which != 3 || !t_h || !t_v)) return LFSR_E_ARG;
   if ((x_stride | x_choff | y_stride | choffH | choffV) & 3) return LFSR_E_ARG;
   if (((uintptr_t)x | (uintptr_t)y | (uintptr_t)w1_planes | (uintptr_t)w2_planes | (uintptr_t)t_h | (uintptr_t)t_v) & 15) return LFSR_E_ARG;
-  if ((long long)B * A * A * h * w * x_stride * 4 >= (1LL << 31) || (long long)B * A * A * h * w * y_stride * 4 >= (1LL << 31)) return LFSR_E_ARG;
+  if ((long long)B * A * A * h * w * x_stride * 4 >= (1LL << 31) || (y && (long long)B * A * A * h * w * y_stride * 4 >= (1LL << 31))) return LFSR_E_ARG;
   if (!(slope >= 0.f && slope <= 1.f)) return LFSR_E_ARG;
   static std::atomic<bool> attr_set[64];
   static std::atomic<int> cus[64];
   int dev = 0;
   if (hipGetDevice(&dev) != hipSuccess || dev < 0 || dev >= 64) return LFSR_E_ARG;
   if (!attr_set[dev]) {
-    hipError_t e = hipFuncSetAttribute(reinterpret_cast<const void*>(k_epi_b3), hipFuncAttributeMaxDynamicSharedMemorySize, EB_SMEM);
+    hipError_t e = hipFuncSetAttribute(reinterpret_cast<const void*>(k_epi_b3<true>), hipFuncAttributeMaxDynamicSharedMemorySize, EB_SMEM);
+    if (e == hipSuccess) e = hipFuncSetAttribute(reinterpret_cast<const void*>(k_epi_b3<false>), hipFuncAttributeMaxDynamicSharedMemorySize, EB_SMEM1);
     if (e != hipSuccess) return LFSR_HIP_ERR(e);
     int v = 0;
     cus[dev] = (hipDeviceGetAttribute(&v, hipDeviceAttributeMultiprocessorCount, dev) == hipSuccess && v > 0) ? v : 256;
@@ -394,7 +404,7 @@
   p.X = x; p.x_stride = x_stride; p.x_choff = x_choff; p.x_bytes = (int)((long long)B * A * A * h * w * x_stride * 4);
   p.W1p = reinterpret_cast<const uint4*>(w1_planes); p.W2p = reinterpret_cast<const uint4*>(w2_planes);
   p.Y = y; p.y_stride = y_stride; p.choffH = choffH; p.choffV = choffV; p.TH = t_h; p.TV = t_v;
-  p.y_bytes = (int)((long long)B * A * A * h * w * y_stride * 4);
+  p.y_bytes = y ? (int)((long long)B * A * A * h * w * y_stride * 4) : 0;
   p.B = B; p.H = h; p.W = w; p.slope = slope;
   p.tilesH = (which & 1) ? (B * A * h + EB_LINES - 1) / EB_LINES : 0;
   p.tilesV = (which & 2) ? (B * A * w + EB_LINES - 1) / EB_LINES : 0;
@@ -403,7 +413,8 @@
   if (which == 3 && (A * h) % EB_LINES == 0 && (A * w) % EB_LINES == 0) { p.tpiH = A * h / EB_LINES; p.tpiV = A * w / EB_LINES; }
   int grid = cus[dev];
   if (grid > ngroups) grid = ngroups;
-  hipLaunchKernelGGL(k_epi_b3, dim3((unsigned)grid), dim3(512), EB_SMEM, st, p);
+  if (y) hipLaunchKernelGGL(k_epi_b3<true>, dim3((unsigned)grid), dim3(512), EB_SMEM, st, p);
+  else hipLaunchKernelGGL(k_epi_b3<false>, dim3((unsigned)grid), dim3(512), EB_SMEM1, st, p);
   LFSR_CHECK_LAUNCH();
   return LFSR_OK;
 }
diff --git a/ntire-2026-light-field-image-super-resolution-challenge---track-2-efficiency_amd/csrc/lfsr_internal.h b/ntire-2026-light-field-image-super-resolution-challenge---track-2-efficiency_amd/csrc/lfsr_internal.h
--- a/ntire-2026-light-field-image-super-resolution-challenge---track-2-efficiency_amd/csrc/lfsr_internal.h
+++ b/ntire-2026-light-field-image-super-resolution-challenge---track-2-efficiency_amd/csrc/lfsr_internal.h
@@ -91,6 +91,10 @@
 int lfsr_epi_b3_launch(const float* x, int x_stride, int x_choff, const float* w1_planes, const float* w2_planes, float* y, int y_stride,
                        int choffH, int choffV, float* t_h, float* t_v, int B, int A, int h, int w, int which, float slope, hipStream_t st);
 int lfsr_pack_epi_wino(const float* w1_direct_packed, float* out, hipStream_t st);
+bool lfsr_distg_tail_ok(int A, int h, int w, const float* x, int x_stride, int x_choff, const float* t_h, const float* t_v);
+int lfsr_distg_tail_launch(const float* spa, int spa_stride, int spa_choff, const float* t_a, const float* t_h, const float* t_v, const float* wa2_packed,
+                           const float* we2_planes, const float* wf_packed, float* y, int y_stride, int y_choff, int B, int A, int h, int w, float slope,
+                           hipStream_t st);
 bool lfsr_epi_fused_ok(int A, int h, int w);
 int lfsr_epi_fused_launch(const float* x, int x_stride, int x_choff, const float* w1_packed, const float* w2_packed, float* y, int y_stride,
                           int choffH, int choffV, float* t_h, float* t_v, int B, int A, int h, int w, int which, float slope, hipStream_t st);
```
